# preshanth/rfi_toolbox

Hardware: AMD Instinct MI355X
Metric: training patches/sec (128x128x3) (higher is better)
Workload: dtype f32; 1 GPU; UNet(3,1,32) train step (fwd+BCE/dice+bwd+clip+Adam), batch 64/GPU x 128x128x3 NHWC, BASELINE configs[1] shape on the reference's U-Net (the '3-layer CNN' of configs[1] is not in the reference; its builder-defined form runs with --workload cnn3); global_batch=64, parallelism=dp1, params=7765985

## Files before the change

rfi_toolbox_amd/build.py:

```python
from __future__ import annotations

import os
import subprocess
import sys
from concurrent.futures import ThreadPoolExecutor

PKG = os.path.dirname(os.path.abspath(__file__))
ROOT = os.path.dirname(PKG)
CSRC = os.path.join(PKG, "csrc")
OBJ = os.path.join(ROOT, "build", "obj")
LIB = os.path.join(PKG, "librfi_hip.so")
HIPCC = os.environ.get("HIPCC", "/opt/rocm/bin/hipcc")
ARCH = "gfx950"

SOURCES = ["api.cpp", "api_ops.cpp", "model.cpp", "model_cnn.cpp", "model_planes.cpp", "model_resnet.cpp", "model_mask.cpp", "model_backbone.cpp", "model_mlp.cpp", "model_params.cpp", "elem_kernels.hip", "conv_direct.hip", "conv_mfma.hip",
           "wgrad_mfma.hip", "preprocess.hip", "synth.hip", "order_stats.hip", "planes_elem.hip", "conv_planes.hip", "conv_ws.hip", "conv_stem.hip", "gemm_ws.hip", "wgrad_ws.hip", "wgrad_stem.hip", "wgrad_planes.hip", "wgrad_split.hip", "detect_kernels.hip", "detect_sample.hip", "detect_infer.hip", "rpn_kernels.hip", "resnet_kernels.hip", "flag_stats.hip", "rfi_sim.hip", "stitch.hip", "dataset_norm.hip", "augment.hip", "sumthreshold.hip"]
HEADERS = ["common.hpp", "kernels.hpp", "model.hpp", "planes.hpp", "ws_common.hpp", "detect_sort.hpp", "select_common.hpp", os.path.join(ROOT, "include", "rfi_hip.h")]

COMMON = ["-O3", "-std=c++17", "-fPIC", f"--offload-arch={ARCH}", "-Wall", "-Wno-unused-function",
          "-ffp-contract=off"]
if os.environ.get("RFI_DIAG_STAMPS"):
    COMMON.append("-DRFI_DIAG_STAMPS=1")


def _newer(target, deps):
    if not os.path.exists(target):
        return True
    t = os.path.getmtime(target)
    return any(os.path.getmtime(d) > t for d in deps)


NO_SLP = {"elem_kernels.hip", "planes_elem.hip", "resnet_kernels.hip", "rpn_kernels.hip", "detect_kernels.hip",
          "preprocess.hip", "order_stats.hip", "synth.hip", "conv_direct.hip", "flag_stats.hip", "dataset_norm.hip", "augment.hip", "sumthreshold.hip",
          "conv_planes.hip", "wgrad_planes.hip", "wgrad_split.hip", "wgrad_mfma.hip", "conv_mfma.hip",
          "conv_ws.hip", "gemm_ws.hip", "wgrad_ws.hip", "conv_stem.hip", "wgrad_stem.hip"}


def flags_for(src):
    return ["-fno-slp-vectorize"] if src in NO_SLP else []


HAZARD_WINDOW = 20


def count_pk_f64_pairs(lines, window=HAZARD_WINDOW):
    import re
    n = 0
    for i, l in enumerate(lines):
        m = re.match(r"v_pk_\w+_f32\s+v\[(\d+):(\d+)\]", l)
        if not m:
            continue
        dst = set(range(int(m.group(1)), int(m.group(2)) + 1))
        for j in range(i + 1, min(i + 1 + window, len(lines))):
            if not dst:
                break
            c = re.match(r"v_cvt_f64_f32\w*\s+v\[\d+:\d+\],\s+v(\d+)", lines[j])
            if c and int(c.group(1)) in dst:
                n += 1
                break
            mv = re.match(r"v_mov_b32\w*\s+v(\d+),\s+v(\d+)\s*$", lines[j])
            copied = mv is not None and int(mv.group(2)) in dst
            w = re.match(r"v_\w+\s+v\[?(\d+)(?::(\d+))?\]?", lines[j])
            if w:
                dst -= set(range(int(w.group(1)), int(w.group(2) or w.group(1)) + 1))
            if copied:
                dst.add(int(mv.group(1)))
    return n


def isa_lines(path):
    return [l.strip() for l in open(path) if l.startswith("\t") and not l.startswith("\t.") and not l.startswith("\t;")]


def _compile(src, force, extra):
    import glob
    path = os.path.join(CSRC, src)
    obj = os.path.join(OBJ, src.replace(".", "_") + ".o")
    deps = [path] + [h if os.path.isabs(h) else os.path.join(CSRC, h) for h in HEADERS]
    if not force and not _newer(obj, deps):
        return obj, None
    device = src.endswith(".hip")
    cmd = [HIPCC, *COMMON, *flags_for(src), *extra, *(["-save-temps=obj"] if device else []), "-x", "hip", "-c", path, "-o", obj]
    r = subprocess.run(cmd, capture_output=True, text=True)
    if r.returncode != 0:
        raise RuntimeError(f"hipcc failed on {src}:\n{' '.join(cmd)}\n{r.stdout}\n{r.stderr}")
    if device:
        stem = os.path.join(OBJ, os.path.splitext(src)[0])
        asm = stem + "-hip-amdgcn-amd-amdhsa-gfx950.s"
        pairs = count_pk_f64_pairs(isa_lines(asm)) if os.path.exists(asm) else -1
        for f in glob.glob(stem + "-hip-amdgcn-amd-amdhsa-gfx950.*") + glob.glob(stem + "-host-x86_64-unknown-linux-gnu.*") + \
                glob.glob(stem + ".hip-hip-amdgcn-amd-amdhsa.hipfb"):
            os.remove(f)
        if pairs != 0:
            os.remove(obj)
            raise RuntimeError(f"{src}: " + ("no device ISA was produced to scan" if pairs < 0 else
                               f"{pairs} packed-fp32 -> v_cvt_f64_f32 pair(s) in the gfx950 ISA (a hazard on MI355X: see NO_SLP above); "
                               "build the source with -fno-slp-vectorize or form the product in float32 first"))
    return obj, r.stderr


# ... 22 lines not shown
```

rfi_toolbox_amd/csrc/conv_ws.hip:

```cpp
#include <algorithm>
#include <type_traits>
#include <vector>

#include <hip/hip_ext.h>

#include "ws_common.hpp"

namespace rfi {
namespace {

using namespace ws;

struct WsDev {
    const float* x;
    int x_ps;
    unsigned x_bytes;
    const float* scale;
    const float* shift;
    float slope;
    int N, H, W, Cin, Cout;
    const bf16_t* wB;
    int nkc, ncb;
    const float* bias;
    float* y;
    int y_ps;
    double* stats;
    int wide_epi;
    unsigned long long* stamps;
};

template <int P> constexpr int ROWB = 32 * P + 16;

template <int TB, int TH, int TW, int NTL, bool ADB, int P>
struct WsCfg {
    static constexpr int HH = TH + 2, HW = TW + 2, HPI = HH * HW, HP = TB * HPI;
    static constexpr int A_BYTES = (HP * ROWB<P> + 1023) & ~1023;
    static constexpr int NPIECE = 9 * NTL * P;
    static constexpr int B_BYTES = NPIECE * 1024;
    static constexpr int B_ITEMS = (NPIECE + 3) / 4;
    static constexpr int HALO_ITEMS = (HP * 4 + 255) / 256;
    static constexpr int B_OFF = (ADB ? 2 : 1) * A_BYTES;
    static constexpr int STAT_OFF = B_OFF + 2 * B_BYTES;
    static constexpr int STAT_BYTES = 4 * NTL * 64 * 2 * 8;
    static constexpr int EPI_WAVE_BYTES = 16 * 36 * 4;
    static constexpr bool WIDE_OK = STAT_OFF + 4 * EPI_WAVE_BYTES <= 160 * 1024;
    static constexpr int LDS_BYTES = STAT_OFF + ((STAT_BYTES > 4 * EPI_WAVE_BYTES || !WIDE_OK) ? STAT_BYTES : 4 * EPI_WAVE_BYTES);
    static_assert(TB * TH * TW == 256, "a tile is 256 output pixels");
    static_assert(32 % TW == 0 || TW % 32 == 0, "a 32-pixel block covers whole rows or a part of one");
    static_assert(LDS_BYTES <= 160 * 1024, "LDS budget");
};


template <int TB, int TH, int TW, int NTL, int XF, bool ADB, int P>
__global__ __launch_bounds__(512) void conv_ws_kernel(WsDev d) {
    using C = WsCfg<TB, TH, TW, NTL, ADB, P>;
    constexpr int RB = ROWB<P>;
    extern __shared__ __attribute__((aligned(16))) unsigned char smem[];
#ifdef RFI_DIAG_STAMPS
    unsigned long long st_[4] = {0, 0, 0, 0};
#endif
    const int tid = threadIdx.x;
    const int lane = tid & 63, wave = __builtin_amdgcn_readfirstlane(tid >> 6);

    const int tiles_x = (d.W + TW - 1) / TW, tiles_y = (d.H + TH - 1) / TH, tiles_b = (d.N + TB - 1) / TB;
    const int ntiles = tiles_b * tiles_y * tiles_x;
    const int GX = gridDim.x;
    int t_begin, t_count, j, gx;
    if (GX >= 8 && (GX & 7) == 0) {
        const int xcd = blockIdx.x & 7, q8 = ntiles >> 3, r8 = ntiles & 7;
        j = blockIdx.x >> 3;
        gx = GX >> 3;
        t_begin = xcd < r8 ? xcd * (q8 + 1) : r8 * (q8 + 1) + (xcd - r8) * q8;
        t_count = q8 + (xcd < r8 ? 1 : 0);
    } else {
        j = blockIdx.x; gx = GX; t_begin = 0; t_count = ntiles;
    }
    const int my_tiles = (j < t_count) ? (t_count - j + gx - 1) / gx : 0;
    const int cb0 = blockIdx.y * NTL, n0 = cb0 * 32;
    double* const st_out = d.stats ? d.stats + ((size_t)blockIdx.x * d.Cout + n0) * 2 : nullptr;
    if (my_tiles == 0) {
        if (st_out && tid < 32 * NTL && n0 + tid < d.Cout) st_out[tid * 2] = st_out[tid * 2 + 1] = 0.0;
        return;
    }
    struct Tile { int n, oy0, ox0; };
    auto tile_of = [&](int k) {
        const int t = t_begin + j + k * gx;
        Tile r;
        r.ox0 = (t % tiles_x) * TW;
        r.oy0 = ((t / tiles_x) % tiles_y) * TH;
        r.n = (t / (tiles_x * tiles_y)) * TB;
        return r;
    };
    const int nkc = d.nkc;
    const int nitems = my_tiles * nkc;
    double* const s_stat = reinterpret_cast<double*>(smem + C::STAT_OFF);

    if (wave >= 4) {
        const int ptid = tid - 256, pw = wave - 4;
        const unsigned q4b = (unsigned)(ptid & 3) * 16u;
        const __amdgpu_buffer_rsrc_t xrs = __builtin_amdgcn_make_buffer_rsrc(const_cast<float*>(d.x), 0, (int)d.x_bytes, 0x00020000);
        unsigned h_rc[C::HALO_ITEMS];
#pragma unroll
        for (int it = 0; it < C::HALO_ITEMS; ++it) {
            const int idx = ptid + it * 256, pix = idx >> 2;
            const int b = pix / C::HPI, rem = pix % C::HPI;
            h_rc[it] = idx < C::HP * 4 ? ((unsigned)b << 24) | ((unsigned)(rem / C::HW) << 12) | (unsigned)(rem % C::HW) : (0xfffu << 12);
        }
        unsigned voff[C::HALO_ITEMS];
        unsigned vmsk[C::HALO_ITEMS];
        auto setup_halo = [&](const Tile& t) {
#pragma unroll
            for (int it = 0; it < C::HALO_ITEMS; ++it) {
                const int n = t.n + (int)(h_rc[it] >> 24);
                const int iy = t.oy0 - 1 + (int)((h_rc[it] >> 12) & 0xfff), ix = t.ox0 - 1 + (int)(h_rc[it] & 0xfff);
                const bool ok = n < d.N && (unsigned)iy < (unsigned)d.H && (unsigned)ix < (unsigned)d.W;
                voff[it] = ok ? (unsigned)(((n * d.H + iy) * d.W + ix) * d.x_ps) * 4u + q4b : 0x80000000u;
                vmsk[it] = ok ? 0xffffffffu : 0u;
            }
        };
        u32x4 raw[C::HALO_ITEMS];
        f32x4 screg = {1.f, 1.f, 1.f, 1.f}, shreg = {0.f, 0.f, 0.f, 0.f};
        unsigned pl[C::HALO_ITEMS][2 * P];
        auto issue_loads = [&](int c0) {
            if constexpr (XF != 0) {
                screg = *reinterpret_cast<const f32x4*>(d.scale + c0 + (ptid & 3) * 4);
                shreg = *reinterpret_cast<const f32x4*>(d.shift + c0 + (ptid & 3) * 4);
            }
            __builtin_amdgcn_sched_barrier(0);
#pragma unroll
            for (int it = 0; it < C::HALO_ITEMS; ++it) raw[it] = __builtin_amdgcn_raw_buffer_load_b128(xrs, voff[it], c0 * 4, 0);
        };
        auto split_all = [&]() {
#pragma unroll
            for (int it = 0; it < C::HALO_ITEMS; ++it) {
                f32x4 v = __builtin_bit_cast(f32x4, raw[it]);
                if constexpr (XF != 0) {
#pragma unroll
                    for (int e = 0; e < 4; ++e) {
                        float t = v[e] * screg[e] + shreg[e];
                        if constexpr (XF == 1) asm("v_max_f32 %0, 0, %1" : "=v"(t) : "v"(t));
                        else t = __builtin_fmaxf(t, t * d.slope);
                        v[e] = __builtin_bit_cast(float, __builtin_bit_cast(unsigned, t) & vmsk[it]);
                    }
                }
                if constexpr (P == 3) {
                    split_pair(v.x, v.y, pl[it][0], pl[it][2], pl[it][4]);
                    split_pair(v.z, v.w, pl[it][1], pl[it][3], pl[it][5]);
                } else {
                    pl[it][0] = cvt_pair(v.x, v.y);
                    pl[it][1] = cvt_pair(v.z, v.w);
                }
            }
        };
        auto write_all = [&](int buf) {
            unsigned char* const sA = smem + buf * C::A_BYTES + (ptid >> 2) * RB + (ptid & 3) * 8;
#pragma unroll
            for (int it = 0; it < C::HALO_ITEMS; ++it) {
                if (ptid + it * 256 < C::HP * 4) {
                    unsigned char* row = sA + it * 64 * RB;
#pragma unroll
                    for (int p = 0; p < P; ++p) *reinterpret_cast<u32x2*>(row + 32 * p) = u32x2{pl[it][2 * p], pl[it][2 * p + 1]};
                }
            }
        };
// ... 253 lines not shown
                                        s_ep[(qi & 1) * 288 + (k + 4 * lh) * 36 + li] = v[0];
                                        s_ep[(qi & 1) * 288 + (k + 1 + 4 * lh) * 36 + li] = v[1];
                                        s1v[nt] += v;
                                        s2v[nt] = __builtin_elementwise_fma(v, v, s2v[nt]);
                                    }
                                }
                                if (qi > 0) {
                                    const int pq = qi - 1, nt = pq >> 3, mt = (pq >> 2) & 1;
                                    const int p = cw * 64 + mt * 32 + (pq & 3) * 8 + pl;
                                    const int b = p / (TH * TW), rr = p % (TH * TW);
                                    *reinterpret_cast<f32x4*>(d.y + tile_off + (unsigned)(((b * d.H + rr / TW) * d.W + rr % TW) * d.y_ps) +
                                                              (unsigned)(n0 + nt * 32 + c4)) = rq;
                                }
                            }
                        } else {
#pragma unroll
                            for (int e = 0; e < E; e += 2) {
                                const int nt = e / 32, mt = (e >> 4) & 1, r = e & 15;
                                const f32x2 v = f32x2{acc[mt][nt][r], acc[mt][nt][r + 1]} + f32x2{bias[nt], bias[nt]};
#pragma unroll
                                for (int k = 0; k < 2; ++k) {
                                    const int p = cw * 64 + mt * 32 + ((r + k) & 3) + 8 * ((r + k) >> 2);
                                    const int b = p / (TH * TW), rr = p % (TH * TW);
                                    d.y[tile_off + (unsigned)(((b * d.H + rr / TW) * d.W + rr % TW) * d.y_ps) + lane_off[nt]] = v[k];
                                }
                                s1v[nt] += v;
                                s2v[nt] = __builtin_elementwise_fma(v, v, s2v[nt]);
                            }
                        }
#pragma unroll
                        for (int nt = 0; nt < NTL; ++nt) {
                            s1[nt] += s1v[nt].x + s1v[nt].y;
                            s2[nt] += s2v[nt].x + s2v[nt].y;
                        }
                    } else {
                        epi_generic(acc, ct);
                    }
                    epi_finish();
                }
                cch = 0;
                ++ck;
                if (ck < my_tiles) ct = tile_of(ck);
            }
            WS_T(t4);
            wg_barrier();
            WS_T(t5);
            WS_ACC(0, t0, t1);
            WS_ACC(2, t1, t4);
            WS_ACC(1, t4, t5);
        }
        if constexpr (DEFER) {
            if (pend) {
                epi_generic(outr, pt);
                epi_finish();
            }
        }
        if (st_out) {
#pragma unroll
            for (int nt = 0; nt < NTL; ++nt) {
                s_stat[((cw * NTL + nt) * 64 + lane) * 2] = d1[nt];
                s_stat[((cw * NTL + nt) * 64 + lane) * 2 + 1] = d2[nt];
            }
        }
    }
#ifdef RFI_DIAG_STAMPS
    if (d.stamps && lane == 0) {
        unsigned long long* o = d.stamps + ((size_t)(blockIdx.y * gridDim.x + blockIdx.x) * 8 + wave) * 8;
        for (int i = 0; i < 4; ++i) o[i] = st_[i];
        o[4] = (unsigned long long)nitems;
    }
#endif
    if (st_out) {
        __syncthreads();
        if (tid < 32 * NTL && n0 + tid < d.Cout) {
            const int nt = tid >> 5, cl = tid & 31;
            double t1 = 0.0, t2 = 0.0;
#pragma unroll
            for (int w = 0; w < 4; ++w)
#pragma unroll
                for (int h = 0; h < 2; ++h) {
                    t1 += s_stat[((w * NTL + nt) * 64 + h * 32 + cl) * 2];
                    t2 += s_stat[((w * NTL + nt) * 64 + h * 32 + cl) * 2 + 1];
                }
            st_out[tid * 2] = t1;
            st_out[tid * 2 + 1] = t2;
        }
    }
}

template <int TB, int TH, int TW, int NTL, int XF, int P>
void launch_ws(rfi_ctx* ctx, ConvArgs& a, WsDev& d) {
    constexpr bool ADB = NTL == 1 || P == 1;
    using C = WsCfg<TB, TH, TW, NTL, ADB, P>;
    const int ntiles = (int)(cdiv(a.N, TB) * cdiv(a.H, TH) * cdiv(a.W, TW));
    const int ycols = (int)cdiv(d.ncb, NTL);
    const int gmax = std::max(8, 256 / ycols);
    const int tx = (int)cdiv(ntiles, 8);
    const int per = (int)cdiv(tx, std::max(1, gmax / 8));
    int GX = 8 * (int)cdiv(tx, per);
    if (ntiles < 8) GX = ntiles;
    if (a.stats && GX <= a.stats_max_records) a.stats_records = GX;
    else { a.stats = nullptr; a.stats_records = 0; }
    d.stats = a.stats;
    static PerDeviceOnce attr_once;
    attr_once.run(ctx->device, [&] {
        RFI_CHECK_HIP(hipFuncSetAttribute(reinterpret_cast<const void*>(&conv_ws_kernel<TB, TH, TW, NTL, XF, ADB, P>),
                                          hipFuncAttributeMaxDynamicSharedMemorySize, (int)C::LDS_BYTES));
    });
#ifdef RFI_DIAG_STAMPS
    {
        const size_t nw = (size_t)GX * ycols * 8;
        RFI_CHECK_HIP(hipMalloc(reinterpret_cast<void**>(&d.stamps), nw * 64));
        RFI_CHECK_HIP(hipMemsetAsync(d.stamps, 0, nw * 64, ctx->stream));
        hipLaunchKernelGGL((conv_ws_kernel<TB, TH, TW, NTL, XF, ADB, P>), dim3(GX, ycols), dim3(512), C::LDS_BYTES, ctx->stream, d);
        std::vector<unsigned long long> hs(nw * 8);
        RFI_CHECK_HIP(hipMemcpyAsync(hs.data(), d.stamps, nw * 64, hipMemcpyDeviceToHost, ctx->stream));
        RFI_CHECK_HIP(hipStreamSynchronize(ctx->stream));
        double c[5] = {0, 0, 0, 0, 0}, p[5] = {0, 0, 0, 0, 0};
        for (size_t w = 0; w < nw; ++w)
            for (int i = 0; i < 5; ++i) ((w & 7) < 4 ? c : p)[i] += (double)hs[w * 8 + i];
        std::fprintf(stderr, "[stamps] conv_ws<%d,%d,%d,%d,%d> N%d %dx%d %d->%d grid %dx%d items/wg %.1f | cycles per item: consumer mfma %.0f "
                     "epilogue %.0f barriers %.0f (+ in front of tap 8: %.0f) | producer work %.0f (split %.0f, dma wait %.0f) barriers+write %.0f\n", TB, TH, TW, NTL, XF,
                     a.N, a.H, a.W, a.Cin, a.Cout, GX, ycols, c[4] / (nw / 2), c[0] / c[4], c[2] / c[4], c[1] / c[4], c[3] / c[4], p[0] / p[4],
                     p[2] / p[4], p[3] / p[4], p[1] / p[4]);
        RFI_CHECK_HIP(hipFree(d.stamps));
        d.stamps = nullptr;
        return;
    }
#endif
    if (a.done) {
        hipExtLaunchKernelGGL((conv_ws_kernel<TB, TH, TW, NTL, XF, ADB, P>), dim3(GX, ycols), dim3(512), C::LDS_BYTES, ctx->stream, nullptr,
                              a.done, 0, d);
        a.done_used = true;
    } else {
        hipLaunchKernelGGL((conv_ws_kernel<TB, TH, TW, NTL, XF, ADB, P>), dim3(GX, ycols), dim3(512), C::LDS_BYTES, ctx->stream, d);
    }
    check_launch("conv_ws");
}

template <int NTL, int XF, int P>
void dispatch_ws(rfi_ctx* ctx, ConvArgs& a, WsDev& d) {
    if (a.W >= 32) launch_ws<1, 8, 32, NTL, XF, P>(ctx, a, d);
    else if (a.W >= 16) launch_ws<1, 16, 16, NTL, XF, P>(ctx, a, d);
    else launch_ws<4, 8, 8, NTL, XF, P>(ctx, a, d);
}
template <int NTL, int P>
void dispatch_xf(rfi_ctx* ctx, ConvArgs& a, WsDev& d, int xf) {
    if (xf == 0) dispatch_ws<NTL, 0, P>(ctx, a, d);
    else if (xf == 1) dispatch_ws<NTL, 1, P>(ctx, a, d);
    else dispatch_ws<NTL, 2, P>(ctx, a, d);
}

}

bool conv_ws_eligible(const ConvArgs& a) {
    if (!(a.R == 3 && a.S == 1 && a.pad == 1 && a.zgroups == 1 && a.fold == 0)) return false;
    if (a.Hin != a.H || a.Win != a.W || a.Hout != a.H || a.Wout != a.W) return false;
    if (a.osy != 1 || a.osx != 1 || a.ooy != 0 || a.oox != 0) return false;
    if (a.y16 || a.W < 8 || a.H < 8) return false;
    if (a.Cin % 16 != 0 || a.x.pstride % 4 != 0 || (reinterpret_cast<uintptr_t>(a.x.p) & 15)) return false;
    if (a.xf.scale && ((reinterpret_cast<uintptr_t>(a.xf.scale) & 15) || (reinterpret_cast<uintptr_t>(a.xf.shift) & 15))) return false;
    if ((int64_t)a.N * a.H * a.W * a.x.pstride * 4 >= (int64_t)1 << 31 || (int64_t)a.N * a.H * a.W * a.y.pstride >= (int64_t)1 << 31) return false;
    return true;
}

void launch_conv_ws(rfi_ctx* ctx, ConvArgs& a, const bf16_t* wB, int P) {
    RFI_REQUIRE(conv_ws_eligible(a), "conv_ws: shape not eligible");
    RFI_REQUIRE(P == 1 || P == 3, "conv_ws: planes must be 1 or 3");
    WsDev d;
    d.x = a.x.p; d.x_ps = a.x.pstride;
    d.x_bytes = (unsigned)((int64_t)a.N * a.H * a.W * a.x.pstride * 4);
    d.scale = a.xf.scale; d.shift = a.xf.shift;
    d.slope = a.xf.relu == 0 ? 1.0f : a.xf.slope;
    d.N = a.N; d.H = a.H; d.W = a.W; d.Cin = a.Cin; d.Cout = a.Cout;
    d.wB = wB;
    d.nkc = plane_chunks(a.Cin); d.ncb = (a.Cout + 31) / 32;
    RFI_REQUIRE((int64_t)wb_elems(9, a.Cout, a.Cin, 0, P) * 2 < ((int64_t)1 << 32), "conv_ws: filter tensor too large");
    d.bias = a.bias;
    d.y = a.y.p; d.y_ps = a.y.pstride;
    d.stats = nullptr;
    d.stamps = nullptr;
    d.wide_epi = a.y.pstride % 4 == 0 && (reinterpret_cast<uintptr_t>(a.y.p) & 15) == 0;
    const int64_t tiles = (a.W >= 16 ? (int64_t)a.N : cdiv(a.N, 4)) * cdiv(a.H, a.W >= 32 ? 8 : a.W >= 16 ? 16 : 8) * cdiv(a.W, a.W >= 32 ? 32 : a.W >= 16 ? 16 : 8);
    int ntl = 1;
    if (a.Cout > 32 && tiles * cdiv(d.ncb, 2) >= 224) ntl = 2;
    if (P == 1 && a.Cout > 64 && tiles * cdiv(d.ncb, 4) >= 224) ntl = 4;
// ... 21 lines not shown
```

rfi_toolbox_amd/csrc/elem_kernels.hip:

```cpp
#include <hip/hip_ext.h>

#include "kernels.hpp"

namespace rfi {

namespace {

constexpr int kBlock = 256;
constexpr int kFinCh = 2;
constexpr int kFinLanes = kBlock / kFinCh;

__device__ __forceinline__ double wave_sum(double v) {
#pragma unroll
    for (int o = 32; o > 0; o >>= 1) v += __shfl_down(v, o, 64);
    return v;
}

__device__ __forceinline__ double finish_sum(double v, double* red) {
#pragma unroll
    for (int o = 32; o >= kFinCh; o >>= 1) v += __shfl_xor(v, o, 64);
    const int wave = threadIdx.x >> 6, lane = threadIdx.x & 63;
    __syncthreads();
    if (lane < kFinCh) red[wave * kFinCh + lane] = v;
    __syncthreads();
    double t = 0;
    if (threadIdx.x < kFinCh)
        for (int w = 0; w < kBlock / 64; ++w) t += red[w * kFinCh + threadIdx.x];
    return t;
}

struct ChanGeom {
    int V;
    int CL, RL, cblocks;
    int64_t rows_per_block;
    int rblocks;
};

static ChanGeom chan_geom(int64_t M, int C, int max_rblocks, bool allow_vec = true, int force_v = 0) {
    ChanGeom g;
    g.V = force_v ? force_v : (allow_vec && C % 4 == 0) ? 4 : 1;
    const int lanes_needed = C / g.V;
    int cl = (g.V >= 4) ? 1 : 4;
    while (cl < lanes_needed && cl < 64) cl <<= 1;
    g.CL = cl;
    g.RL = kBlock / cl;
    g.cblocks = (int)cdiv(lanes_needed, cl);
    int64_t rpb = cdiv(M, max_rblocks);
    int64_t min_rows = (int64_t)g.RL * 8;
    if (rpb < min_rows) rpb = min_rows;
    rpb = cdiv(rpb, g.RL) * g.RL;
    g.rows_per_block = rpb;
    g.rblocks = (int)cdiv(M, rpb);
    return g;
}

template <int V>
__device__ __forceinline__ void ldv(const float* p, float (&v)[V]) {
    if constexpr (V == 4) {
        const float4 t = *reinterpret_cast<const float4*>(p);
        v[0] = t.x; v[1] = t.y; v[2] = t.z; v[3] = t.w;
    } else {
        v[0] = p[0];
    }
}
template <int V>
__device__ __forceinline__ void stv(float* p, const float (&v)[V]) {
    if constexpr (V == 4) *reinterpret_cast<float4*>(p) = make_float4(v[0], v[1], v[2], v[3]);
    else p[0] = v[0];
}
template <int V>
__device__ __forceinline__ void ldy(const void* y, int y16, int64_t idx, float (&v)[V]) {
    if (y16) {
        const unsigned short* q = static_cast<const unsigned short*>(y) + idx;
        if constexpr (V == 4) {
            const uint2 t = *reinterpret_cast<const uint2*>(q);
            v[0] = __builtin_bit_cast(float, t.x << 16); v[1] = __builtin_bit_cast(float, t.x & 0xffff0000u);
            v[2] = __builtin_bit_cast(float, t.y << 16); v[3] = __builtin_bit_cast(float, t.y & 0xffff0000u);
        } else {
            v[0] = __builtin_bit_cast(float, (unsigned)q[0] << 16);
        }
    } else {
        ldv<V>(static_cast<const float*>(y) + idx, v);
    }
}
__device__ __forceinline__ float ldy1(const void* y, int y16, int64_t idx) {
    float v[1];
    ldy<1>(y, y16, idx, v);
    return v[0];
}
__device__ __forceinline__ void round_store_bf16x4(unsigned short* p, float (&v)[4]) {
    unsigned short q[4];
#pragma unroll
    for (int e = 0; e < 4; ++e) {
        const __bf16 h = (__bf16)v[e];
        q[e] = __builtin_bit_cast(unsigned short, h);
        v[e] = (float)h;
    }
    *reinterpret_cast<uint2*>(p) = make_uint2((unsigned)q[0] | ((unsigned)q[1] << 16), (unsigned)q[2] | ((unsigned)q[3] << 16));
}
template <int V, int NQ>
__device__ __forceinline__ void row_lane_reduce(double (&acc)[NQ][V], double* red, int CL, int RL, int cl,
                                                int rl) {
#pragma unroll
// ... 18 lines not shown
                acc[q][v] = t0 + t1;
            }
    }
    if (NF > 1) {
        __syncthreads();
        if (rl > 0 && rl < NF) {
#pragma unroll
            for (int q = 0; q < NQ; ++q)
#pragma unroll
                for (int v = 0; v < V; ++v) red[(q * V + v) * kBlock + threadIdx.x] = acc[q][v];
        }
        __syncthreads();
        if (rl == 0) {
#pragma unroll
            for (int q = 0; q < NQ; ++q)
#pragma unroll
                for (int v = 0; v < V; ++v) {
                    double t = acc[q][v];
                    for (int j = 1; j < NF; ++j) t += red[(q * V + v) * kBlock + j * CL + cl];
                    acc[q][v] = t;
                }
        }
    }
}

__device__ __forceinline__ float act_f(float a, float slope) { return a > 0.0f ? a : (slope != 0.0f ? a * slope : 0.0f); }
__device__ __forceinline__ float dact_f(float z, float g, float slope) { return z > 0.0f ? g : g * slope; }

template <int V>
__global__ void bn_stats_kernel(const float* __restrict__ y, int64_t M, int C, int CL,
                                int64_t rows_per_block, double* __restrict__ partial) {
    __shared__ double red[2 * V * kBlock];
    const int RL = kBlock / CL;
    const int cl = threadIdx.x % CL, rl = threadIdx.x / CL;
    const int c = (blockIdx.y * CL + cl) * V;
    const int64_t r0 = (int64_t)blockIdx.x * rows_per_block;
    int64_t r1 = r0 + rows_per_block;
    if (r1 > M) r1 = M;
    double acc[2][V];
#pragma unroll
    for (int v = 0; v < V; ++v) acc[0][v] = acc[1][v] = 0;
    if (c < C) {
        for (int64_t r = r0 + rl; r < r1; r += RL) {
            float x[V];
            ldv<V>(y + r * C + c, x);
#pragma unroll
            for (int v = 0; v < V; ++v) {
                const double d = (double)x[v];
                acc[0][v] += d;
                acc[1][v] += d * d;
            }
        }
    }
    row_lane_reduce<V, 2>(acc, red, CL, RL, cl, rl);
    if (rl == 0 && c < C) {
#pragma unroll
        for (int v = 0; v < V; ++v) {
            partial[((int64_t)blockIdx.x * C + c + v) * 2 + 0] = acc[0][v];
            partial[((int64_t)blockIdx.x * C + c + v) * 2 + 1] = acc[1][v];
        }
    }
}

__global__ void bn_finalize_kernel(const double* __restrict__ partial, int records, int C,
                                   double count, const float* __restrict__ gamma,
                                   const float* __restrict__ beta, float* __restrict__ running_mean,
                                   float* __restrict__ running_var, int ema_repeats,
                                   float* __restrict__ mean_out, float* __restrict__ invstd_out,
                                   float* __restrict__ scale, float* __restrict__ shift,
                                   float* __restrict__ var_out) {
    __shared__ double red[2 * kBlock];
    const int cl = threadIdx.x & (kFinCh - 1), rl = threadIdx.x / kFinCh;
    const int c = blockIdx.x * kFinCh + cl;
    double s1 = 0, s2 = 0;
    if (c < C) {
        for (int r = rl; r < records; r += kFinLanes) {
            s1 += partial[((int64_t)r * C + c) * 2 + 0];
            s2 += partial[((int64_t)r * C + c) * 2 + 1];
        }
    }
    s1 = finish_sum(s1, red);
    s2 = finish_sum(s2, red);
    if (rl == 0 && c < C) {
        const double mean = s1 / count;
        double var = s2 / count - mean * mean;
        if (var < 0) var = 0;
        const double invstd = 1.0 / sqrt(var + 1e-5);
        const float meanf = (float)mean, invf = (float)invstd;
        mean_out[c] = meanf;
        invstd_out[c] = invf;
        if (var_out) var_out[c] = (float)var;
        const float sc = gamma[c] * invf;
        scale[c] = sc;
        shift[c] = beta[c] - meanf * sc;
        if (running_mean) {
            const double var_u = count > 1 ? var * (count / (count - 1.0)) : var;
            float rm = running_mean[c], rv = running_var[c];
            const float vuf = (float)var_u;
            for (int k = 0; k < ema_repeats; ++k) {
                rm = (1.0f - 0.1f) * rm + 0.1f * meanf;
                rv = (1.0f - 0.1f) * rv + 0.1f * vuf;
            }
            running_mean[c] = rm;
            running_var[c] = rv;
        }
    }
}

__global__ void bn_eval_coeffs_kernel(int C, const float* gamma, const float* beta, const float* rm,
                                      const float* rv, float* scale, float* shift) {
    int c = blockIdx.x * blockDim.x + threadIdx.x;
    if (c < C) {
        float inv = (float)(1.0 / sqrt((double)rv[c] + 1e-5));
        float sc = gamma[c] * inv;
        scale[c] = sc;
        shift[c] = beta[c] - rm[c] * sc;
    }
}

template <int V>
__global__ void bn_bwd_reduce_kernel(const void* __restrict__ da, int da16, const void* __restrict__ y, int y16, int64_t yps,
                                     int64_t M, int C, int CL, int64_t rows_per_block,
                                     const float* __restrict__ scale, const float* __restrict__ shift,
                                     const float* __restrict__ mean, const float* __restrict__ invstd,
                                     double* __restrict__ partial, float slope) {
    __shared__ double red[2 * V * kBlock];
    const int RL = kBlock / CL;
    const int cl = threadIdx.x % CL, rl = threadIdx.x / CL;
    const int c = (blockIdx.y * CL + cl) * V;
    const int64_t r0 = (int64_t)blockIdx.x * rows_per_block;
    int64_t r1 = r0 + rows_per_block;
    if (r1 > M) r1 = M;
    double acc[2][V];
#pragma unroll
    for (int v = 0; v < V; ++v) acc[0][v] = acc[1][v] = 0;
    if (c < C) {
        float sc[V], sh[V], mu[V], is[V];
        ldv<V>(scale + c, sc); ldv<V>(shift + c, sh); ldv<V>(mean + c, mu); ldv<V>(invstd + c, is);
        constexpr int U = 4;
        for (int64_t rb = r0 + rl; rb < r1; rb += (int64_t)U * RL) {
            float yv[U][V], dv[U][V];
#pragma unroll
            for (int k = 0; k < U; ++k) {
                const int64_t r = rb + (int64_t)k * RL;
                if (r < r1) {
                    ldy<V>(y, y16, r * yps + c, yv[k]);
                    ldy<V>(da, da16, r * C + c, dv[k]);
                }
            }
#pragma unroll
            for (int k = 0; k < U; ++k) {
                if (rb + (int64_t)k * RL < r1) {
#pragma unroll
                    for (int v = 0; v < V; ++v) {
                        const float dz = dact_f(yv[k][v] * sc[v] + sh[v], dv[k][v], slope);
                        const float xh = (yv[k][v] - mu[v]) * is[v];
                        acc[0][v] += (double)dz;
                        acc[1][v] += (double)dz * (double)xh;
                    }
                }
            }
        }
    }
    row_lane_reduce<V, 2>(acc, red, CL, RL, cl, rl);
    if (rl == 0 && c < C) {
#pragma unroll
        for (int v = 0; v < V; ++v) {
            partial[((int64_t)blockIdx.x * C + c + v) * 2 + 0] = acc[0][v];
            partial[((int64_t)blockIdx.x * C + c + v) * 2 + 1] = acc[1][v];
        }
    }
}

__device__ __forceinline__ void ld8h(const unsigned short* p, float (&v)[8]) {
    const uint4 t = *reinterpret_cast<const uint4*>(p);
    v[0] = __builtin_bit_cast(float, t.x << 16); v[1] = __builtin_bit_cast(float, t.x & 0xffff0000u);
    v[2] = __builtin_bit_cast(float, t.y << 16); v[3] = __builtin_bit_cast(float, t.y & 0xffff0000u);
    v[4] = __builtin_bit_cast(float, t.z << 16); v[5] = __builtin_bit_cast(float, t.z & 0xffff0000u);
    v[6] = __builtin_bit_cast(float, t.w << 16); v[7] = __builtin_bit_cast(float, t.w & 0xffff0000u);
}
__device__ __forceinline__ void ld8f(const float* p, float (&v)[8]) {
    const float4 a = *reinterpret_cast<const float4*>(p), b = *reinterpret_cast<const float4*>(p + 4);
    v[0] = a.x; v[1] = a.y; v[2] = a.z; v[3] = a.w; v[4] = b.x; v[5] = b.y; v[6] = b.z; v[7] = b.w;
}
__device__ __forceinline__ unsigned pack_bf16x2(float a, float b) {
    const __bf16 ha = (__bf16)a, hb = (__bf16)b;
    return (unsigned)__builtin_bit_cast(unsigned short, ha) | ((unsigned)__builtin_bit_cast(unsigned short, hb) << 16);
}
// ... 433 lines not shown
            if ((int)threadIdx.x < C4) {
#pragma unroll
                for (int v = 0; v < 4; ++v) {
                    double t1 = 0.0, t2 = 0.0;
                    for (int k = threadIdx.x; k < kBlock; k += C4) {
                        t1 += red[(2 * v) * kBlock + k];
                        t2 += red[(2 * v + 1) * kBlock + k];
                    }
                    records[((int64_t)blockIdx.x * C + c + v) * 2 + 0] = t1;
                    records[((int64_t)blockIdx.x * C + c + v) * 2 + 1] = t2;
                }
            }
        } else {
            const int per = C4 / kBlock;
#pragma unroll
            for (int v = 0; v < 4; ++v) {
                records[((int64_t)(blockIdx.x / per) * C + c + v) * 2 + 0] = s1[v];
                records[((int64_t)(blockIdx.x / per) * C + c + v) * 2 + 1] = s2[v];
            }
        }
    }
}

__global__ void copy_edge_kernel(int N, int H, int W, int C, const float* __restrict__ dskip,
                                 int dskip_ps, float* __restrict__ da) {
    const int64_t total = (int64_t)N * H * W * C;
    const int He = H & ~1, We = W & ~1;
    for (int64_t i = (int64_t)blockIdx.x * blockDim.x + threadIdx.x; i < total;
         i += (int64_t)gridDim.x * blockDim.x) {
        const int c = (int)(i % C);
        const int64_t pix = i / C;
        const int x = (int)(pix % W);
        const int yy = (int)((pix / W) % H);
        if (yy >= He || x >= We) da[pix * C + c] = dskip[pix * dskip_ps + c];
    }
}

__global__ void head_fwd_kernel(const float* __restrict__ y, int64_t M, int C,
                                const float* __restrict__ scale, const float* __restrict__ shift,
                                const float* __restrict__ w, const float* __restrict__ b, int Cout,
                                float* __restrict__ logits, float slope) {
    const int lane16 = threadIdx.x & 15;
    const int64_t m = ((int64_t)blockIdx.x * blockDim.x + threadIdx.x) >> 4;
    if (m >= M) return;
    for (int o = 0; o < Cout; ++o) {
        float acc = 0.0f;
        for (int c = lane16; c < C; c += 16) {
            float a = y[m * C + c] * scale[c] + shift[c];
            a = act_f(a, slope);
            acc += a * w[o * C + c];
        }
#pragma unroll
        for (int off = 8; off > 0; off >>= 1) acc += __shfl_down(acc, off, 16);
        if (lane16 == 0) logits[m * Cout + o] = acc + b[o];
    }
}

template <int L>
__global__ __launch_bounds__(256) void head_fwd_vec_kernel(const void* __restrict__ y, int y16, int64_t yps, int64_t M, int C,
                                                           const float* __restrict__ scale, const float* __restrict__ shift,
                                                           const float* __restrict__ w, const float* __restrict__ b, int Cout,
                                                           float* __restrict__ logits, float slope) {
    const int lane = threadIdx.x & (L - 1);
    const int64_t m = ((int64_t)blockIdx.x * blockDim.x + threadIdx.x) / L;
    if (m >= M) return;
    const int C4 = C >> 2;
    for (int o = 0; o < Cout; ++o) {
        float acc = 0.0f;
        for (int c4 = lane; c4 < C4; c4 += L) {
            float yv[4], sc[4], sh[4], wv[4];
            ldy<4>(y, y16, m * yps + 4 * c4, yv); ldv<4>(scale + 4 * c4, sc); ldv<4>(shift + 4 * c4, sh);
            ldv<4>(w + (int64_t)o * C + 4 * c4, wv);
#pragma unroll
            for (int v = 0; v < 4; ++v) acc += act_f(yv[v] * sc[v] + sh[v], slope) * wv[v];
        }
#pragma unroll
        for (int off = L / 2; off > 0; off >>= 1) acc += __shfl_down(acc, off, L);
        if (lane == 0) logits[m * Cout + o] = acc + b[o];
    }
}

__device__ __forceinline__ float sigmoidf_(float x) { return 1.0f / (1.0f + expf(-x)); }

__global__ void loss_reduce_kernel(const float* __restrict__ logits, const uint8_t* __restrict__ labels,
                                   int64_t count, double* __restrict__ partial) {
    __shared__ double red[4][kBlock / 64];
    double s[4] = {0, 0, 0, 0};
    for (int64_t i = (int64_t)blockIdx.x * blockDim.x + threadIdx.x; i < count;
         i += (int64_t)gridDim.x * blockDim.x) {
        const float x = logits[i];
        const float t = labels[i] ? 1.0f : 0.0f;
        const float bce = fmaxf(x, 0.0f) - x * t + log1pf(expf(-fabsf(x)));
        const float p = sigmoidf_(x);
        s[0] += (double)bce;
        s[1] += (double)(p * t);
        s[2] += (double)p;
        s[3] += (double)t;
    }
    const int wave = threadIdx.x >> 6, lane = threadIdx.x & 63;
#pragma unroll
    for (int k = 0; k < 4; ++k) {
        double v = wave_sum(s[k]);
        if (lane == 0) red[k][wave] = v;
    }
    __syncthreads();
    if (threadIdx.x < 4) {
        double v = 0;
        for (int wv = 0; wv < kBlock / 64; ++wv) v += red[threadIdx.x][wv];
        partial[(int64_t)blockIdx.x * 4 + threadIdx.x] = v;
    }
}

__global__ void loss_finish_kernel(const double* __restrict__ partial, int blocks, double count,
                                   double* __restrict__ sums4, float* __restrict__ loss_out) {
    __shared__ double red[4][kBlock / 64];
    double s[4] = {0, 0, 0, 0};
    for (int b = threadIdx.x; b < blocks; b += blockDim.x)
        for (int k = 0; k < 4; ++k) s[k] += partial[(int64_t)b * 4 + k];
    const int wave = threadIdx.x >> 6, lane = threadIdx.x & 63;
#pragma unroll
    for (int k = 0; k < 4; ++k) {
        double v = wave_sum(s[k]);
        if (lane == 0) red[k][wave] = v;
    }
    __syncthreads();
    if (threadIdx.x == 0) {
        double t[4];
        for (int k = 0; k < 4; ++k) {
            t[k] = 0;
            for (int wv = 0; wv < kBlock / 64; ++wv) t[k] += red[k][wv];
            sums4[k] = t[k];
        }
        const float bce = (float)(t[0] / count);
        const float inter = (float)t[1], sp = (float)t[2], st = (float)t[3];
        const float dice = 1.0f - (2.0f * inter + 1.0f) / (sp + st + 1.0f);
        loss_out[0] = bce + dice;
    }
}

__global__ void loss_bwd_kernel(const float* __restrict__ logits, const uint8_t* __restrict__ labels,
                                int64_t count, const double* __restrict__ sums4,
                                float* __restrict__ dlogits) {
    const float inter = (float)sums4[1], sp = (float)sums4[2], st = (float)sums4[3];
    const float D = sp + st + 1.0f;
    const float num = 2.0f * inter + 1.0f;
    const float invD2 = 1.0f / (D * D);
    const float invN = (float)(1.0 / (double)count);
    for (int64_t i = (int64_t)blockIdx.x * blockDim.x + threadIdx.x; i < count;
         i += (int64_t)gridDim.x * blockDim.x) {
        const float x = logits[i];
        const float t = labels[i] ? 1.0f : 0.0f;
        const float p = sigmoidf_(x);
        const float ddice = -(2.0f * t * D - num) * invD2;
        dlogits[i] = (p - t) * invN + ddice * p * (1.0f - p);
    }
}

__device__ __forceinline__ float focal_elem(float x, float t, float alpha, float gamma) {
    const float p = sigmoidf_(x);
    const float ce = fmaxf(x, 0.0f) - x * t + log1pf(expf(-fabsf(x)));
    const float pt = p * t + (1.0f - p) * (1.0f - t);
    const float at = alpha >= 0.0f ? alpha * t + (1.0f - alpha) * (1.0f - t) : 1.0f;
    return at * powf(1.0f - pt, gamma) * ce;
}
__global__ void focal_reduce_kernel(const float* __restrict__ logits, const uint8_t* __restrict__ labels,
                                    int64_t count, float alpha, float gamma, double* __restrict__ partial) {
    __shared__ double red[kBlock / 64];
    double s = 0;
    for (int64_t i = (int64_t)blockIdx.x * blockDim.x + threadIdx.x; i < count; i += (int64_t)gridDim.x * blockDim.x)
        s += (double)focal_elem(logits[i], labels[i] ? 1.0f : 0.0f, alpha, gamma);
    s = wave_sum(s);
    if ((threadIdx.x & 63) == 0) red[threadIdx.x >> 6] = s;
    __syncthreads();
    if (threadIdx.x == 0) {
        double t = 0;
        for (int k = 0; k < kBlock / 64; ++k) t += red[k];
        partial[blockIdx.x] = t;
    }
}
__global__ void focal_finish_kernel(const double* __restrict__ partial, int blocks, double count,
                                    float* __restrict__ loss_out) {
    __shared__ double red[kBlock / 64];
    double s = 0;
    for (int b = threadIdx.x; b < blocks; b += blockDim.x) s += partial[b];
    s = wave_sum(s);
    if ((threadIdx.x & 63) == 0) red[threadIdx.x >> 6] = s;
    __syncthreads();
    if (threadIdx.x == 0) {
        double t = 0;
        for (int k = 0; k < kBlock / 64; ++k) t += red[k];
        loss_out[0] = (float)(t / count);
    }
}
__global__ void focal_bwd_kernel(const float* __restrict__ logits, const uint8_t* __restrict__ labels, int64_t count,
                                 float alpha, float gamma, float* __restrict__ dlogits) {
    const float invN = (float)(1.0 / (double)count);
    for (int64_t i = (int64_t)blockIdx.x * blockDim.x + threadIdx.x; i < count; i += (int64_t)gridDim.x * blockDim.x) {
        const float x = logits[i];
        const bool pos = labels[i] != 0;
        const float p = sigmoidf_(x);
        const float sp_neg = fmaxf(-x, 0.0f) + log1pf(expf(-fabsf(x)));
        const float sp_pos = fmaxf(x, 0.0f) + log1pf(expf(-fabsf(x)));
        float g;
        if (pos) {
            const float a = alpha >= 0.0f ? alpha : 1.0f;
            g = a * powf(1.0f - p, gamma) * (gamma * p * (-sp_neg) - (1.0f - p));
        } else {
            const float a = alpha >= 0.0f ? 1.0f - alpha : 1.0f;
            g = a * powf(p, gamma) * (p - gamma * (1.0f - p) * (-sp_pos));
        }
        dlogits[i] = g * invN;
    }
}

__global__ void sigmoid_fwd_kernel(const float* __restrict__ z, int64_t n, float* __restrict__ x) {
    for (int64_t i = (int64_t)blockIdx.x * blockDim.x + threadIdx.x; i < n; i += (int64_t)gridDim.x * blockDim.x)
        x[i] = sigmoidf_(z[i]);
}
__global__ void sigmoid_bwd_kernel(const float* __restrict__ x, int64_t n, float* __restrict__ d) {
    for (int64_t i = (int64_t)blockIdx.x * blockDim.x + threadIdx.x; i < n; i += (int64_t)gridDim.x * blockDim.x) {
// ... 169 lines not shown
    }
}
__global__ void nhwc_to_nchw_kernel(const float* __restrict__ src, int N, int C, int H, int W,
                                    float* __restrict__ dst) {
    const int64_t total = (int64_t)N * C * H * W;
    for (int64_t i = (int64_t)blockIdx.x * blockDim.x + threadIdx.x; i < total;
         i += (int64_t)gridDim.x * blockDim.x) {
        const int x = (int)(i % W);
        int64_t t = i / W;
        const int yy = (int)(t % H);
        t /= H;
        const int c = (int)(t % C);
        const int n = (int)(t / C);
        dst[i] = src[(((int64_t)n * H + yy) * W + x) * C + c];
    }
}
__global__ void weight_to_dgrad_kernel(const float* __restrict__ wf, int taps, int Cout, int Cin,
                                       int flip, float* __restrict__ wd) {
    const int64_t total = (int64_t)taps * Cout * Cin;
    for (int64_t i = (int64_t)blockIdx.x * blockDim.x + threadIdx.x; i < total;
         i += (int64_t)gridDim.x * blockDim.x) {
        const int co = (int)(i % Cout);
        int64_t t = i / Cout;
        const int ci = (int)(t % Cin);
        const int tp = (int)(t / Cin);
        const int ts = flip ? (taps - 1 - tp) : tp;
        wd[i] = wf[((int64_t)ts * Cout + co) * Cin + ci];
    }
}
__global__ __launch_bounds__(256) void weight_to_dgrad_batched_kernel(const RelayoutDesc* __restrict__ descs, int n,
                                                                     const float* __restrict__ src, float* __restrict__ dst) {
    __shared__ float tile[32][33];
    const int64_t b = blockIdx.x;
    int l = 0;
    while (l + 1 < n && descs[l + 1].tile0 <= b) ++l;
    const RelayoutDesc d = descs[l];
    const float* __restrict__ wf = src + d.src_off;
    float* __restrict__ wd = dst + d.dst_off;
    const int tci = (d.cin + 31) / 32, tco = (d.cout + 31) / 32;
    const int t = (int)(b - d.tile0);
    const int tp = t / (tci * tco), r = t % (tci * tco);
    const int bco = r / tci, bci = r % tci;
    const int ts = d.flip ? (d.taps - 1 - tp) : tp;
    const int tx = threadIdx.x & 31, ty = threadIdx.x >> 5;
#pragma unroll
    for (int k = 0; k < 4; ++k) {
        const int co = bco * 32 + ty + 8 * k, ci = bci * 32 + tx;
        if (co < d.cout && ci < d.cin) tile[ty + 8 * k][tx] = wf[((int64_t)ts * d.cout + co) * d.cin + ci];
    }
    __syncthreads();
#pragma unroll
    for (int k = 0; k < 4; ++k) {
        const int ci = bci * 32 + ty + 8 * k, co = bco * 32 + tx;
        if (co < d.cout && ci < d.cin) wd[((int64_t)tp * d.cin + ci) * d.cout + co] = tile[tx][ty + 8 * k];
    }
}
__global__ void relu_bwd_kernel(float4* __restrict__ dA, const float4* __restrict__ Y, int64_t n4) {
    for (int64_t i = (int64_t)blockIdx.x * blockDim.x + threadIdx.x; i < n4;
         i += (int64_t)gridDim.x * blockDim.x) {
        float4 g = dA[i];
        const float4 y = Y[i];
        g.x = y.x > 0.0f ? g.x : 0.0f;
        g.y = y.y > 0.0f ? g.y : 0.0f;
        g.z = y.z > 0.0f ? g.z : 0.0f;
        g.w = y.w > 0.0f ? g.w : 0.0f;
        dA[i] = g;
    }
}
__global__ void pad_channels_kernel(const float* __restrict__ s, int64_t M, int c, int cp,
                                    float* __restrict__ d) {
    const int64_t total = M * cp;
    for (int64_t i = (int64_t)blockIdx.x * blockDim.x + threadIdx.x; i < total;
         i += (int64_t)gridDim.x * blockDim.x) {
        const int k = (int)(i % cp);
        d[i] = k < c ? s[(i / cp) * c + k] : 0.0f;
    }
}
__global__ void u8_to_f32_kernel(const uint8_t* __restrict__ s, int64_t n, float* __restrict__ d) {
    for (int64_t i = (int64_t)blockIdx.x * blockDim.x + threadIdx.x; i < n;
         i += (int64_t)gridDim.x * blockDim.x)
        d[i] = (float)s[i];
}

__global__ void sumsq_kernel(const float* __restrict__ g, int64_t n, double* __restrict__ partial) {
    __shared__ double red[kBlock / 64];
    double s = 0;
    const int64_t n4 = n >> 2;
    const float4* g4 = reinterpret_cast<const float4*>(g);
    for (int64_t i = (int64_t)blockIdx.x * blockDim.x + threadIdx.x; i < n4;
         i += (int64_t)gridDim.x * blockDim.x) {
        const float4 v = g4[i];
        s += (double)v.x * v.x + (double)v.y * v.y + (double)v.z * v.z + (double)v.w * v.w;
    }
    if (blockIdx.x == 0 && threadIdx.x < (n & 3)) {
        const float v = g[(n4 << 2) + threadIdx.x];
        s += (double)v * v;
    }
    s = wave_sum(s);
    if ((threadIdx.x & 63) == 0) red[threadIdx.x >> 6] = s;
    __syncthreads();
    if (threadIdx.x == 0) {
        double t = 0;
        for (int k = 0; k < kBlock / 64; ++k) t += red[k];
        partial[blockIdx.x] = t;
    }
}
__global__ void sumsq_finish_kernel(const double* __restrict__ partial, int blocks,
                                    double* __restrict__ out) {
    __shared__ double red[kBlock / 64];
    double s = 0;
    for (int b = threadIdx.x; b < blocks; b += blockDim.x) s += partial[b];
    s = wave_sum(s);
    if ((threadIdx.x & 63) == 0) red[threadIdx.x >> 6] = s;
    __syncthreads();
    if (threadIdx.x == 0) {
        double t = 0;
        for (int k = 0; k < kBlock / 64; ++k) t += red[k];
        out[0] = t;
    }
}

__global__ void adam_kernel(AdamArgs a) {
    const float norm = (float)sqrt(a.sumsq[0]) * a.grad_scale;
    float coef = a.max_norm / (norm + 1e-6f);
    coef = coef > 1.0f ? 1.0f : coef;
    if (a.max_norm <= 0.0f) coef = 1.0f;
    const float gs = a.grad_scale;
    for (int64_t i = (int64_t)blockIdx.x * blockDim.x + threadIdx.x; i < a.n;
         i += (int64_t)gridDim.x * blockDim.x) {
        const float p = a.p[i];
        float g = (a.g[i] * gs) * coef;
        g = __fmaf_rn(a.wd, p, g);
        const float m0 = a.m[i];
        const float m = __fmaf_rn(a.one_minus_beta1, g - m0, m0);
        const float v = __fmaf_rn(a.one_minus_beta2 * g, g, a.beta2 * a.v[i]);
        a.m[i] = m;
        a.v[i] = v;
        const float denom = sqrtf(v) / a.bc2_sqrt + a.eps;
        a.p[i] = p + (a.neg_step * m) / denom;
    }
    if (blockIdx.x == 0 && threadIdx.x == 0 && a.norm_out) a.norm_out[0] = norm;
}

__global__ void scale_inplace_kernel(float* __restrict__ x, int64_t n, float f) {
    for (int64_t i = (int64_t)blockIdx.x * blockDim.x + threadIdx.x; i < n; i += (int64_t)gridDim.x * blockDim.x) x[i] *= f;
}
__global__ void reduce_slabs_kernel(const float* __restrict__ slabs, int nslabs, int group, int kstride,
                                    int64_t n, float* __restrict__ out, int64_t out_rowstride) {
    const int base = blockIdx.y * group;
    int cnt = nslabs - base;
    if (cnt > group) cnt = group;
    for (int64_t i = (int64_t)blockIdx.x * blockDim.x + threadIdx.x; i < n;
         i += (int64_t)gridDim.x * blockDim.x) {
        float s = 0.0f;
        for (int k = 0; k < cnt; ++k) s += slabs[((int64_t)base + (int64_t)k) * kstride * n + i];
        out[(int64_t)blockIdx.y * out_rowstride * n + i] = s;
    }
}

__global__ __launch_bounds__(256) void reduce_slabs_vec4_kernel(const float* __restrict__ slabs, int nslabs, int group, int kstride,
                                                               int64_t n4, float* __restrict__ out, int64_t out_rowstride) {
    typedef float f32x4 __attribute__((ext_vector_type(4)));
    const int base = blockIdx.y * group;
    int cnt = nslabs - base;
    if (cnt > group) cnt = group;
    const f32x4* __restrict__ src = reinterpret_cast<const f32x4*>(slabs) + (int64_t)base * kstride * n4;
    f32x4* __restrict__ dst = reinterpret_cast<f32x4*>(out) + (int64_t)blockIdx.y * out_rowstride * n4;
    const int64_t step = (int64_t)kstride * n4;
    for (int64_t i = (int64_t)blockIdx.x * blockDim.x + threadIdx.x; i < n4; i += (int64_t)gridDim.x * blockDim.x) {
        f32x4 s = {0.f, 0.f, 0.f, 0.f};
        int k = 0;
        for (; k + 8 <= cnt; k += 8) {
            f32x4 v[8];
#pragma unroll
            for (int u = 0; u < 8; ++u) v[u] = __builtin_nontemporal_load(src + (int64_t)(k + u) * step + i);
#pragma unroll
            for (int u = 0; u < 8; ++u) s += v[u];
        }
        for (; k < cnt; ++k) s += __builtin_nontemporal_load(src + (int64_t)k * step + i);
        dst[i] = s;
    }
}

static int grid_for(int64_t total, int cap = 256 * 16) {
    int64_t b = cdiv(total, kBlock);
    if (b > cap) b = cap;
    if (b < 1) b = 1;
    return (int)b;
}

constexpr int kMaxRowBlocks = 1024;

}
// ... 223 lines not shown
           !((reinterpret_cast<uintptr_t>(y.p) | reinterpret_cast<uintptr_t>(scale) | reinterpret_cast<uintptr_t>(shift) |
              reinterpret_cast<uintptr_t>(dskip.p) | reinterpret_cast<uintptr_t>(dpool) | reinterpret_cast<uintptr_t>(da)) & 15);
}
int launch_pool_bwd_merge_sums(rfi_ctx* ctx, YRef y, int N, int H, int W, int C, const float* scale,
                               const float* shift, const float* mean, const float* invstd, YRef dskip, YRef dpool,
                               float* da, float slope, float* partial_ws, unsigned short* da16) {
    if (!pool_vec_ok(y, C, scale, shift, dskip, dpool, da16 ? reinterpret_cast<const float*>(da16) : da) || dpool.stride(C) != C ||
        (reinterpret_cast<uintptr_t>(da16) & 7) ||
        ((reinterpret_cast<uintptr_t>(mean) | reinterpret_cast<uintptr_t>(invstd)) & 15))
        return 0;
    const int C4 = C / 4;
    const int64_t total = (int64_t)N * (H / 2) * (W / 2) * C4;
    const bool small = C4 <= kBlock && kBlock % C4 == 0, wide = C4 > kBlock && C4 % kBlock == 0;
    if ((H & 1) || (W & 1) || !(small || wide) || total < (int64_t)kBlock * 16) return 0;
    int grid = grid_for(total, kMaxRowBlocks);
    int records = grid;
    if (wide) {
        const int per = C4 / kBlock;
        grid = std::max(per, grid / per * per);
        records = grid / per;
    }
    if ((int64_t)grid * kBlock > total) return 0;
    ProfScope ps(ctx, FAM_ELEMWISE, 0, (double)N * H * W * C * (y.bf16 ? 10 : 12) + (double)total * (dpool.bf16 ? 8 : 16));
    hipLaunchKernelGGL(pool_bwd_merge_vec_kernel<true>, dim3(grid), dim3(kBlock), 0, ctx->stream, y.p, y.bf16, y.stride(C), N, H, W,
                       C, scale, shift, mean, invstd, dskip.p, dskip.bf16, (int)dskip.stride(C), dpool.p, dpool.bf16, da, slope, reinterpret_cast<double*>(partial_ws), da16);
    check_launch("pool_bwd_merge_sums");
    return records;
}

void launch_pool_bwd_merge(rfi_ctx* ctx, YRef y, int N, int H, int W, int C,
                           const float* scale, const float* shift, YRef dskip, YRef dpool,
                           float* da, float slope, unsigned short* da16) {
    const bool vec = pool_vec_ok(y, C, scale, shift, dskip, dpool, da16 ? reinterpret_cast<const float*>(da16) : da) && dpool.stride(C) == C &&
                     !(reinterpret_cast<uintptr_t>(da16) & 7);
    RFI_REQUIRE(vec || !(dpool.bf16 || da16 || dskip.bf16), "pool_bwd_merge: bfloat16 gradient tensors need C % 4 == 0 and aligned tensors");
    RFI_REQUIRE(!dskip.bf16 || !((H & 1) || (W & 1)), "pool_bwd_merge: a bfloat16 skip gradient needs even H and W");
    RFI_REQUIRE(!da16 || !((H & 1) || (W & 1)), "pool_bwd_merge: a bfloat16 output needs even H and W");
    const int64_t total = (int64_t)N * (H / 2) * (W / 2) * C;
    {
        ProfScope ps(ctx, FAM_ELEMWISE, 0, (double)N * H * W * C * (y.bf16 ? 10 : 12) + (double)total * (dpool.bf16 ? 2 : 4));
        if (vec)
            hipLaunchKernelGGL(pool_bwd_merge_vec_kernel<false>, dim3(grid_for(total / 4)), dim3(kBlock), 0, ctx->stream, y.p, y.bf16,
                               y.stride(C), N, H, W, C, scale, shift, nullptr, nullptr, dskip.p, dskip.bf16, (int)dskip.stride(C), dpool.p, dpool.bf16, da, slope, nullptr, da16);
        else
            hipLaunchKernelGGL(pool_bwd_merge_kernel, dim3(grid_for(total)), dim3(kBlock), 0, ctx->stream, y.p, y.bf16, y.stride(C),
                               N, H, W, C, scale, shift, static_cast<const float*>(dskip.p), (int)dskip.stride(C), static_cast<const float*>(dpool.p), da, slope);
        check_launch("pool_bwd_merge");
    }
    if ((H & 1) || (W & 1)) {
        ProfScope ps(ctx, FAM_ELEMWISE);
        hipLaunchKernelGGL(copy_edge_kernel, dim3(grid_for((int64_t)N * H * W * C)), dim3(kBlock), 0,
                           ctx->stream, N, H, W, C, static_cast<const float*>(dskip.p), (int)dskip.stride(C), da);
        check_launch("copy_edge");
    }
}

void launch_head_fwd(rfi_ctx* ctx, YRef yr, int64_t M, int C, const float* scale,
                     const float* shift, const float* w, const float* b, int Cout, float* logits, float slope) {
    ProfScope ps(ctx, FAM_ELEMWISE, 2.0 * M * C * Cout, (double)M * C * (yr.bf16 ? 2 : 4) + (double)M * Cout * 4);
    const bool vec = C % 4 == 0 && !((reinterpret_cast<uintptr_t>(yr.p) | reinterpret_cast<uintptr_t>(scale) |
                                      reinterpret_cast<uintptr_t>(shift) | reinterpret_cast<uintptr_t>(w)) & 15) && yr.stride(C) % 4 == 0;
    RFI_REQUIRE(vec || !yr.bf16, "head_fwd: a bfloat16 input needs C % 4 == 0");
    const float* y = static_cast<const float*>(yr.p);
    if (vec) {
        int L = 1;
        while (L * 2 <= C / 4 && L < 16) L *= 2;
        const unsigned blocks = (unsigned)cdiv(M * L, kBlock);
#define RFI_HF(L_) hipLaunchKernelGGL(head_fwd_vec_kernel<L_>, dim3(blocks), dim3(kBlock), 0, ctx->stream, yr.p, yr.bf16, yr.stride(C), M, C, scale, shift, w, b, Cout, logits, slope)
        if (L == 16) RFI_HF(16); else if (L == 8) RFI_HF(8); else if (L == 4) RFI_HF(4); else if (L == 2) RFI_HF(2); else RFI_HF(1);
#undef RFI_HF
    } else {
        const int64_t threads = M * 16;
        hipLaunchKernelGGL(head_fwd_kernel, dim3((unsigned)cdiv(threads, kBlock)), dim3(kBlock), 0,
                           ctx->stream, y, M, C, scale, shift, w, b, Cout, logits, slope);
    }
    check_launch("head_fwd");
}

size_t loss_ws_doubles(int64_t count) {
    (void)count;
    return 4 * 1024 + 8;
}
void launch_loss_reduce(rfi_ctx* ctx, const float* logits, const uint8_t* labels, int64_t count,
                        double* partial_ws, double* sums4, float* loss_out) {
    int blocks = grid_for(count, 1024);
    {
        ProfScope ps(ctx, FAM_ELEMWISE, 0, (double)count * 5);
        hipLaunchKernelGGL(loss_reduce_kernel, dim3(blocks), dim3(kBlock), 0, ctx->stream, logits, labels,
                           count, partial_ws);
        check_launch("loss_reduce");
    }
    {
        ProfScope ps(ctx, FAM_ELEMWISE);
        hipLaunchKernelGGL(loss_finish_kernel, dim3(1), dim3(kBlock), 0, ctx->stream, partial_ws, blocks,
                           (double)count, sums4, loss_out);
        check_launch("loss_finish");
    }
}
void launch_focal_reduce(rfi_ctx* ctx, const float* logits, const uint8_t* labels, int64_t count, float alpha,
                         float gamma, double* partial_ws, float* loss_out) {
    int blocks = grid_for(count, 1024);
    {
        ProfScope ps(ctx, FAM_ELEMWISE, 0, (double)count * 5);
        hipLaunchKernelGGL(focal_reduce_kernel, dim3(blocks), dim3(kBlock), 0, ctx->stream, logits, labels, count,
                           alpha, gamma, partial_ws);
        check_launch("focal_reduce");
    }
    {
        ProfScope ps(ctx, FAM_ELEMWISE);
        hipLaunchKernelGGL(focal_finish_kernel, dim3(1), dim3(kBlock), 0, ctx->stream, partial_ws, blocks,
                           (double)count, loss_out);
        check_launch("focal_finish");
    }
}
void launch_focal_bwd(rfi_ctx* ctx, const float* logits, const uint8_t* labels, int64_t count, float alpha,
                      float gamma, float* dlogits) {
    ProfScope ps(ctx, FAM_ELEMWISE, 0, (double)count * 9);
    hipLaunchKernelGGL(focal_bwd_kernel, dim3(grid_for(count)), dim3(kBlock), 0, ctx->stream, logits, labels,
                       count, alpha, gamma, dlogits);
    check_launch("focal_bwd");
}
void launch_loss_bwd(rfi_ctx* ctx, const float* logits, const uint8_t* labels, int64_t count,
                     const double* sums4, float* dlogits) {
    ProfScope ps(ctx, FAM_ELEMWISE, 0, (double)count * 9);
    hipLaunchKernelGGL(loss_bwd_kernel, dim3(grid_for(count)), dim3(kBlock), 0, ctx->stream, logits,
                       labels, count, sums4, dlogits);
    check_launch("loss_bwd");
}

void launch_sigmoid_fwd(rfi_ctx* ctx, const float* z, int64_t n, float* x) {
    ProfScope ps(ctx, FAM_ELEMWISE, 0, (double)n * 8);
    hipLaunchKernelGGL(sigmoid_fwd_kernel, dim3(grid_for(n)), dim3(kBlock), 0, ctx->stream, z, n, x);
    check_launch("sigmoid_fwd");
}
void launch_sigmoid_bwd(rfi_ctx* ctx, const float* x, int64_t n, float* d_inout) {
    ProfScope ps(ctx, FAM_ELEMWISE, 0, (double)n * 12);
    hipLaunchKernelGGL(sigmoid_bwd_kernel, dim3(grid_for(n)), dim3(kBlock), 0, ctx->stream, x, n, d_inout);
    check_launch("sigmoid_bwd");
}

size_t head_bwd_ws_floats(int64_t M, int C, int Cout) {
    (void)M;
    return (size_t)kMaxRowBlocks * ((size_t)Cout * C + Cout) * 2;
}
int launch_head_bwd(rfi_ctx* ctx, YRef yr, int64_t M, int C, const float* scale,
                    const float* shift, const float* w, int Cout, const float* dlogits, float* da,
                    float* partial_ws, float* dw, float* db, float slope, const float* bn_mean, const float* bn_invstd,
                    float* bn_records_ws, unsigned short* da16, bool* skip_da, bool finish) {
    const bool may_skip = skip_da && *skip_da;
    if (skip_da) *skip_da = false;
    int bn_records = 0;
    const bool vec = C % 4 == 0 && !((reinterpret_cast<uintptr_t>(yr.p) | reinterpret_cast<uintptr_t>(da) |
                                      reinterpret_cast<uintptr_t>(scale) | reinterpret_cast<uintptr_t>(shift) |
                                      reinterpret_cast<uintptr_t>(w)) & 15) && yr.stride(C) % 4 == 0;
    RFI_REQUIRE(vec || !yr.bf16, "head_bwd: a bfloat16 input needs C % 4 == 0");
    RFI_REQUIRE(finish || vec, "head_bwd: deferred finishing needs the vector path (C % 4 == 0, 16-byte aligned tensors)");
    RFI_REQUIRE(!da16 || (vec && Cout == 1 && !(reinterpret_cast<uintptr_t>(da16) & 7)), "head_bwd: a bfloat16 gradient tensor needs C % 4 == 0 and one output channel");
    const float* y = static_cast<const float*>(yr.p);
    ChanGeom g = geom_rows(M, C, vec);
    {
        ProfScope ps(ctx, FAM_ELEMWISE, 4.0 * M * C * Cout, (double)M * C * (yr.bf16 ? 6 : 8));
        if (vec) {
            const bool sums = bn_records_ws && bn_mean && bn_invstd && Cout == 1 &&
                              !((reinterpret_cast<uintptr_t>(bn_mean) | reinterpret_cast<uintptr_t>(bn_invstd)) & 15);
            hipLaunchKernelGGL(head_bwd_vec_kernel, dim3(g.rblocks, g.cblocks), dim3(kBlock), 0, ctx->stream, yr.p, yr.bf16,
                               yr.stride(C), M, C, g.CL, g.rows_per_block, scale, shift, w, Cout, dlogits, da,
                               reinterpret_cast<double*>(partial_ws), slope, bn_mean, bn_invstd,
                               sums ? reinterpret_cast<double*>(bn_records_ws) : nullptr, da16, (sums && may_skip && !da16) ? 0 : 1);
            if (sums) bn_records = g.rblocks;
            if (sums && may_skip && !da16) *skip_da = true;
        }
        else
            hipLaunchKernelGGL(head_bwd_kernel, dim3(g.rblocks, g.cblocks), dim3(kBlock), 0, ctx->stream, y,
                               M, C, g.CL, g.rows_per_block, scale, shift, w, Cout, dlogits, da,
                               reinterpret_cast<double*>(partial_ws), slope);
        check_launch("head_bwd");
    }
    if (finish) {
        const int n = Cout * C + Cout;
        ProfScope ps(ctx, FAM_REDUCE);
        hipLaunchKernelGGL(finish_channel_sum_kernel, dim3((int)cdiv(Cout * C, kFinCh)), dim3(kBlock), 0,
                           ctx->stream, reinterpret_cast<const double*>(partial_ws), g.rblocks, (int64_t)n, Cout * C, dw);
        check_launch("head_bwd_finish_dw");
    }
    if (finish) {
        const int n = Cout * C + Cout;
        ProfScope ps(ctx, FAM_REDUCE);
        hipLaunchKernelGGL(finish_channel_sum_kernel, dim3((int)cdiv(Cout, kFinCh)), dim3(kBlock), 0,
                           ctx->stream, reinterpret_cast<const double*>(partial_ws) + (size_t)Cout * C,
                           g.rblocks, (int64_t)n, Cout, db);
        check_launch("head_bwd_finish_db");
    }
    return bn_records;
}

void launch_nchw_to_nhwc(rfi_ctx* ctx, const float* src, int N, int C, int H, int W, float* dst) {
    const int64_t total = (int64_t)N * C * H * W;
    ProfScope ps(ctx, FAM_ELEMWISE, 0, (double)total * 8);
    hipLaunchKernelGGL(nchw_to_nhwc_kernel, dim3(grid_for(total)), dim3(kBlock), 0, ctx->stream, src, N,
                       C, H, W, dst);
    check_launch("nchw_to_nhwc");
}
void launch_nhwc_to_nchw(rfi_ctx* ctx, const float* src, int N, int C, int H, int W, float* dst) {
    const int64_t total = (int64_t)N * C * H * W;
    ProfScope ps(ctx, FAM_ELEMWISE, 0, (double)total * 8);
    hipLaunchKernelGGL(nhwc_to_nchw_kernel, dim3(grid_for(total)), dim3(kBlock), 0, ctx->stream, src, N,
                       C, H, W, dst);
    check_launch("nhwc_to_nchw");
}
void launch_weight_to_dgrad(rfi_ctx* ctx, const float* wf, int taps, int Cout, int Cin, int flip,
                            float* wd) {
    const int64_t total = (int64_t)taps * Cout * Cin;
    ProfScope ps(ctx, FAM_ELEMWISE, 0, (double)total * 8);
    hipLaunchKernelGGL(weight_to_dgrad_kernel, dim3(grid_for(total)), dim3(kBlock), 0, ctx->stream, wf,
                       taps, Cout, Cin, flip, wd);
    check_launch("weight_to_dgrad");
}
int64_t relayout_assign_tiles(RelayoutDesc* descs, int n) {
    int64_t t = 0;
    for (int i = 0; i < n; ++i) {
        descs[i].tile0 = t;
        t += (int64_t)descs[i].taps * ((descs[i].cout + 31) / 32) * ((descs[i].cin + 31) / 32);
    }
    return t;
}
void launch_weight_to_dgrad_batched(rfi_ctx* ctx, const RelayoutDesc* descs_dev, int n, const float* src,
                                    float* dst, double total_bytes, int64_t total_tiles) {
    RFI_REQUIRE(total_tiles > 0 && total_tiles < ((int64_t)1 << 31), "weight_to_dgrad_batched: bad tile count");
    ProfScope ps(ctx, FAM_ELEMWISE, 0, total_bytes);
    hipLaunchKernelGGL(weight_to_dgrad_batched_kernel, dim3((unsigned)total_tiles), dim3(256), 0, ctx->stream, descs_dev, n,
                       src, dst);
    check_launch("weight_to_dgrad_batched");
}
void launch_relu_bwd(rfi_ctx* ctx, float* dA, const float* Y, int64_t n) {
    RFI_REQUIRE(n % 4 == 0, "relu_bwd: element count must be a multiple of 4");
    ProfScope ps(ctx, FAM_ELEMWISE, 0, (double)n * 12);
    hipLaunchKernelGGL(relu_bwd_kernel, dim3(grid_for(n / 4)), dim3(kBlock), 0, ctx->stream,
                       reinterpret_cast<float4*>(dA), reinterpret_cast<const float4*>(Y), n / 4);
    check_launch("relu_bwd");
}
void launch_pad_channels(rfi_ctx* ctx, const float* src, int64_t M, int c, int cp, float* dst) {
    ProfScope ps(ctx, FAM_ELEMWISE, 0, (double)M * (c + cp) * 4);
    hipLaunchKernelGGL(pad_channels_kernel, dim3(grid_for(M * cp)), dim3(kBlock), 0, ctx->stream, src, M, c,
                       cp, dst);
    check_launch("pad_channels");
}
void launch_u8_to_f32(rfi_ctx* ctx, const uint8_t* src, int64_t n, float* dst) {
    ProfScope ps(ctx, FAM_ELEMWISE, 0, (double)n * 5);
    hipLaunchKernelGGL(u8_to_f32_kernel, dim3(grid_for(n)), dim3(kBlock), 0, ctx->stream, src, n, dst);
    check_launch("u8_to_f32");
}

size_t sumsq_ws_doubles(int64_t n) {
    (void)n;
    return 1024 + 8;
}
void launch_sumsq(rfi_ctx* ctx, const float* g, int64_t n, double* partial_ws, double* sumsq) {
    int blocks = grid_for(n / 4 + 1, 1024);
    {
        ProfScope ps(ctx, FAM_OPTIM, 0, (double)n * 4);
        hipLaunchKernelGGL(sumsq_kernel, dim3(blocks), dim3(kBlock), 0, ctx->stream, g, n, partial_ws);
        check_launch("sumsq");
    }
    {
        ProfScope ps(ctx, FAM_OPTIM);
        hipLaunchKernelGGL(sumsq_finish_kernel, dim3(1), dim3(kBlock), 0, ctx->stream, partial_ws, blocks,
                           sumsq);
        check_launch("sumsq_finish");
    }
}
void launch_adam(rfi_ctx* ctx, const AdamArgs& a) {
    ProfScope ps(ctx, FAM_OPTIM, 0, (double)a.n * 28);
    hipLaunchKernelGGL(adam_kernel, dim3(grid_for(a.n)), dim3(kBlock), 0, ctx->stream, a);
    check_launch("adam");
}

void launch_scale_inplace(rfi_ctx* ctx, float* x, int64_t n, float f) {
    if (n <= 0) return;
    ProfScope ps(ctx, FAM_COMM, 0, (double)n * 8);
    hipLaunchKernelGGL(scale_inplace_kernel, dim3(grid_for(n)), dim3(kBlock), 0, ctx->stream, x, n, f);
    check_launch("scale_inplace");
}
void launch_reduce_slabs(rfi_ctx* ctx, const float* slabs, int nslabs, int64_t n, float* out) {
    float* s = const_cast<float*>(slabs);
    int count = nslabs;
    int stride = 1;
    const bool vec = n % 4 == 0 && !((reinterpret_cast<uintptr_t>(slabs) | reinterpret_cast<uintptr_t>(out)) & 15);
    while (count > 32) {
        const int groups = (int)cdiv(count, 32);
        ProfScope ps(ctx, FAM_REDUCE, 0, (double)n * 4 * (count + groups));
        if (vec)
            hipLaunchKernelGGL(reduce_slabs_vec4_kernel, dim3(grid_for(n / 4, 1024), groups), dim3(kBlock), 0, ctx->stream, s, count, 32,
                               stride, n / 4, s, (int64_t)32 * stride);
        else
        hipLaunchKernelGGL(reduce_slabs_kernel, dim3(grid_for(n, 1024), groups), dim3(kBlock), 0,
                           ctx->stream, s, count, 32, stride, n, s, (int64_t)32 * stride);
        check_launch("reduce_slabs_fold");
        count = groups;
        stride *= 32;
    }
    ProfScope ps(ctx, FAM_REDUCE, 0, (double)n * 4 * (count + 1));
    if (vec)
        hipLaunchKernelGGL(reduce_slabs_vec4_kernel, dim3(grid_for(n / 4, 1024), 1), dim3(kBlock), 0, ctx->stream, s, count, 32, stride,
                           n / 4, out, (int64_t)0);
    else
    hipLaunchKernelGGL(reduce_slabs_kernel, dim3(grid_for(n, 1024), 1), dim3(kBlock), 0, ctx->stream, s,
                       count, 32, stride, n, out, (int64_t)0);
    check_launch("reduce_slabs");
}

}
```

rfi_toolbox_amd/csrc/kernels.hpp:

```cpp
#pragma once
#include "common.hpp"

namespace rfi {

struct InXform {
    const float* scale = nullptr;
    const float* shift = nullptr;
    int relu = 0;
    float slope = 0.0f;
};
static inline InXform act_xform(const float* scale, const float* shift, float slope) {
    return InXform{scale, shift, slope != 0.0f ? 2 : 1, slope};
}

struct View {
    const float* p = nullptr;
    int pstride = 0;
};
struct MutView {
    float* p = nullptr;
    int pstride = 0;
};

struct ConvArgs {
    View x;
    int N = 0, H = 0, W = 0;
    int Hin = 0, Win = 0;
    int Cin = 0, Cout = 0;
    const float* w = nullptr;
    const float* w3 = nullptr;
    const unsigned short* wB3 = nullptr;
    const unsigned short* wB1 = nullptr;
    const float* bias = nullptr;
    MutView y;
    int Hout = 0, Wout = 0;
    int osy = 1, osx = 1;
    int ooy = 0, oox = 0;
    int R = 3, S = 1, pad = 1;
    int zgroups = 1;
    unsigned short* y16 = nullptr;
    int fold = 0;
    InXform xf;
    double algo_flops = -1;
    bool bf16 = false;
    bool bf16x3 = false;
    int planes = 0;
    double* stats = nullptr;
    int stats_max_records = 0;
    int stats_records = 0;
    hipEvent_t done = nullptr;
    bool done_used = false;
#ifdef RFI_DIAG_STAMPS
    unsigned long long* stamps = nullptr;
#endif
};

enum ConvImpl { IMPL_AUTO = 0, IMPL_DIRECT = 1, IMPL_MFMA = 2, IMPL_MFMA_BF16 = 3, IMPL_MFMA_BF16X3 = 4,
                IMPL_PLANES_X3 = 5, IMPL_PLANES_BF16 = 6, IMPL_WS_X3 = 7, IMPL_WS_BF16 = 8 };
bool conv_ws_eligible(const ConvArgs& a);
void launch_conv_ws(rfi_ctx* ctx, ConvArgs& a, const unsigned short* wB, int P);
bool gemm_ws_eligible(const ConvArgs& a);
void launch_gemm_ws(rfi_ctx* ctx, ConvArgs& a, const unsigned short* wB3);

bool conv_mfma_eligible(const ConvArgs& a);
size_t weights_x3_floats(int taps, int Cout, int Cin);
void launch_weights_to_x3(rfi_ctx* ctx, const float* w, int taps, int Cout, int Cin, float* out);
struct X3Desc { const float* src; float* dst; int64_t rows; int Cin; int nchunks; };
void launch_weights_to_x3_batched(rfi_ctx* ctx, const X3Desc* descs_dev, int n, double total_bytes);
bool conv_stem_eligible(const ConvArgs& a);
void launch_conv_stem(rfi_ctx* ctx, ConvArgs& a);
void launch_conv(rfi_ctx* ctx, ConvArgs& a, int impl = IMPL_AUTO);

struct WgradArgs {
    View xop, yop;
    InXform xf_x, xf_y;
    int N = 0, H = 0, W = 0;
    int Hx = 0, Wx = 0;
    int Cx = 0, Cy = 0;
    int R = 3, S = 1, pad = 1;
    float* dw = nullptr;
    int64_t tap_stride = 0;
    int sy = 0, sx = 0;
    float* slab = nullptr;
    size_t slab_floats = 0;
    double algo_flops = -1;
    bool bf16 = false;
    bool bf16x3 = false;
    int planes = 0;
};
size_t wgrad_slab_floats(const WgradArgs& a, int impl);
bool wgrad_ws_eligible(const WgradArgs& a);
void launch_wgrad_ws(rfi_ctx* ctx, const WgradArgs& a);
size_t wgrad_ws_slab_floats(const WgradArgs& a);
bool wgrad_stem_eligible(const WgradArgs& a);
void launch_wgrad_stem(rfi_ctx* ctx, const WgradArgs& a);
void launch_wgrad(rfi_ctx* ctx, const WgradArgs& a, int impl = IMPL_AUTO);

struct YRef {
    const void* p = nullptr;
    int bf16 = 0;
    int64_t ps = 0;
    YRef(const float* f) : p(f) {}
    YRef(float* f) : p(f) {}
    YRef(const float* f, int64_t pstride) : p(f), ps(pstride) {}
    YRef(const unsigned short* h, int64_t pstride) : p(h), bf16(1), ps(pstride) {}
    YRef(View v) : p(v.p), ps(v.pstride) {}
    int64_t stride(int C) const { return ps ? ps : C; }
};

size_t bn_stats_ws_floats(int C);
void launch_bn_stats(rfi_ctx* ctx, const float* y, int64_t M, int C, float* partial_ws);
void launch_bn_finalize(rfi_ctx* ctx, const float* partial_ws, int64_t M, int C, const float* gamma,
                        const float* beta, float* running_mean, float* running_var,
                        int ema_repeats, float* mean, float* invstd, float* scale, float* shift,
                        float* var_out, int records = 0,
                        hipEvent_t done = nullptr);
void launch_bn_eval_coeffs(rfi_ctx* ctx, int C, const float* gamma, const float* beta,
                           const float* running_mean, const float* running_var, float* scale,
                           float* shift);
void launch_bn_bwd_reduce(rfi_ctx* ctx, YRef da, YRef y, int64_t M, int C,
                          const float* scale, const float* shift, const float* mean,
                          const float* invstd, float* partial_ws, float* c1, float* c2,
                          float* dgamma, float* dbeta, float slope = 0.0f);
size_t bn_bwd_ws_floats(int64_t M, int C);
void launch_bn_bwd_finalize_records(rfi_ctx* ctx, const float* partial_ws, int records, int64_t M, int C, float* c1,
                                    float* c2, float* dgamma, float* dbeta);
void launch_bn_bwd_apply(rfi_ctx* ctx, YRef da_inout, YRef y, int64_t M, int C,
                         const float* scale, const float* shift, const float* mean,
                         const float* invstd, const float* gamma, const float* c1, const float* c2,
                         float* partial_ws, float* dbias, float slope = 0.0f,
                         unsigned short* planes_out = nullptr, int64_t planes_pstride = 0, int planes_P = 0,
                         hipEvent_t done = nullptr, bool finish_dbias = true, const float* head_dl = nullptr,
                         const float* head_w = nullptr);
void launch_bn_bwd_apply_finish(rfi_ctx* ctx, const float* partial_ws, int64_t M, int C, float* dbias);
struct FinishSumDesc { const double* partial; int records; int64_t stride; int count; float* out; };
int bn_bwd_apply_records(int64_t M, int C);
void launch_finish_channel_sums_batched(rfi_ctx* ctx, const FinishSumDesc* descs_dev, int n, int max_count);

void launch_bn_relu_pool(rfi_ctx* ctx, const float* y, int N, int H, int W, int C,
                         const float* scale, const float* shift, MutView skip, float* pooled, float slope = 0.0f);
void launch_pool_bwd_merge(rfi_ctx* ctx, YRef y, int N, int H, int W, int C,
                           const float* scale, const float* shift, YRef dskip, YRef dpool,
                           float* da, float slope = 0.0f, unsigned short* da16 = nullptr);
int launch_pool_bwd_merge_sums(rfi_ctx* ctx, YRef y, int N, int H, int W, int C, const float* scale,
                               const float* shift, const float* mean, const float* invstd, YRef dskip, YRef dpool,
                               float* da, float slope, float* partial_ws, unsigned short* da16 = nullptr);
void launch_head_fwd(rfi_ctx* ctx, YRef y, int64_t M, int C, const float* scale,
                     const float* shift, const float* w, const float* b, int Cout, float* logits,
                     float slope = 0.0f);
void launch_sigmoid_fwd(rfi_ctx* ctx, const float* z, int64_t n, float* x);
void launch_sigmoid_bwd(rfi_ctx* ctx, const float* x, int64_t n, float* d_inout);
void launch_loss_reduce(rfi_ctx* ctx, const float* logits, const uint8_t* labels, int64_t count,
                        double* partial_ws, double* sums4, float* loss_out);
size_t loss_ws_doubles(int64_t count);
void launch_loss_bwd(rfi_ctx* ctx, const float* logits, const uint8_t* labels, int64_t count,
                     const double* sums4, float* dlogits);
void launch_focal_reduce(rfi_ctx* ctx, const float* logits, const uint8_t* labels, int64_t count, float alpha,
                         float gamma, double* partial_ws, float* loss_out);
void launch_focal_bwd(rfi_ctx* ctx, const float* logits, const uint8_t* labels, int64_t count, float alpha,
                      float gamma, float* dlogits);
int launch_head_bwd(rfi_ctx* ctx, YRef y, int64_t M, int C, const float* scale,
                    const float* shift, const float* w, int Cout, const float* dlogits, float* da,
                    float* partial_ws, float* dw, float* db, float slope = 0.0f, const float* bn_mean = nullptr,
                    const float* bn_invstd = nullptr, float* bn_records_ws = nullptr, unsigned short* da16 = nullptr,
                    bool* skip_da = nullptr, bool finish = true);
size_t head_bwd_ws_floats(int64_t M, int C, int Cout);
void launch_channel_sum(rfi_ctx* ctx, View v, int64_t M, int C, float* partial_ws, float* out, bool finish = true);
void launch_channel_sum(rfi_ctx* ctx, YRef v, int64_t M, int C, float* partial_ws, float* out, bool finish = true);
size_t channel_sum_ws_floats(int64_t M, int C);

void launch_nchw_to_nhwc(rfi_ctx* ctx, const float* src, int N, int C, int H, int W, float* dst);
void launch_nhwc_to_nchw(rfi_ctx* ctx, const float* src, int N, int C, int H, int W, float* dst);
void launch_weight_to_dgrad(rfi_ctx* ctx, const float* wf, int taps, int Cout, int Cin, int flip,
                            float* wd);
struct RelayoutDesc {
    int64_t src_off, dst_off;
    int taps, cout, cin, flip;
    int64_t tile0 = 0;
};
int64_t relayout_assign_tiles(RelayoutDesc* descs, int n);
void launch_weight_to_dgrad_batched(rfi_ctx* ctx, const RelayoutDesc* descs_dev, int n, const float* src,
                                    float* dst, double total_bytes, int64_t total_tiles);
void launch_u8_to_f32(rfi_ctx* ctx, const uint8_t* src, int64_t n, float* dst);
void launch_relu_bwd(rfi_ctx* ctx, float* dA, const float* Y, int64_t n);
void launch_pad_channels(rfi_ctx* ctx, const float* src, int64_t M, int c, int cp, float* dst);

void launch_sumsq(rfi_ctx* ctx, const float* g, int64_t n, double* partial_ws, double* sumsq);
size_t sumsq_ws_doubles(int64_t n);
struct AdamArgs {
    float* p; float* g; float* m; float* v; int64_t n;
    float beta2, eps, wd, max_norm, grad_scale;
    float one_minus_beta1, one_minus_beta2;
    float neg_step, bc2_sqrt;
    const double* sumsq;
    float* norm_out;
};
void launch_adam(rfi_ctx* ctx, const AdamArgs& a);

void launch_preprocess(rfi_ctx* ctx, const void* patches, int dtype, int n, int ph, int pw,
                       float* minmax_ws, float* out_nhwc, const rfi_patch_src* table_dev = nullptr, int C = 0,
                       int T = 0);
void launch_patch_median(rfi_ctx* ctx, const double* v, int n, int per, bool absdev, const double* centre,
                         bool finite_only, double* out, int* cnt_out, bool f32 = false);
void launch_scale_by_median(rfi_ctx* ctx, double* v, int n, int per, const double* med, bool f32 = false);
void launch_stretch(rfi_ctx* ctx, double* v, int64_t total, int kind, bool f32 = false);
void launch_replace_inf(rfi_ctx* ctx, double* v, int n, int per, const double* mad, const int* nfinite);
void launch_mad_flags(rfi_ctx* ctx, const double* v, int n, int per, const double* med, const double* mad,
                      double sigma, uint8_t* flags, bool f32 = false);
void launch_narrow_f32(rfi_ctx* ctx, const double* src, int64_t total, float* dst);
void launch_to_abs_f64(rfi_ctx* ctx, const void* src, int dtype, int64_t total, double* dst);
void launch_synth(rfi_ctx* ctx, unsigned long long seed, int n_samples, int n_pol, int C, int T, double noise,
                  int bandpass, int order, double corr, const rfi_event* events_dev, const int* offsets_dev,
                  int out_dtype, void* planes, uint8_t* flags);
void launch_gather_labels(rfi_ctx* ctx, const uint8_t* flags, const rfi_patch_src* table_dev, int C, int T, int n,
                          int ps, uint8_t* out);
void launch_patch_any_flag(rfi_ctx* ctx, const uint8_t* flags, const rfi_patch_src* table_dev, int C, int T, int n,
                           int ps, unsigned* any_out);
void launch_confusion(rfi_ctx* ctx, const void* pred, int pred_dtype, const void* truth,
                      int truth_dtype, int64_t count, unsigned long long* counts3);
void launch_threshold(rfi_ctx* ctx, const float* logits, int64_t count, float threshold,
                      uint8_t* mask);
int64_t tiling_patches_per_plane(int C, int T, const rfi_tiling& tiling);
void check_tiling(const rfi_tiling& tiling);
void launch_stitch(rfi_ctx* ctx, const float* values, int kind, int n_planes, int C, int T, const rfi_tiling& tiling,
                   int combine, float threshold, uint8_t* flags, float* prob);
size_t flag_stats_ws_bytes();
void launch_flag_stats(rfi_ctx* ctx, const void* src, int dtype, int64_t n, const uint8_t* flags, int views,
                       bool medians, void* ws, void* mag, rfi_flag_stats* out_dev);
struct norm_chunk { const void* ptr; int64_t start; };
size_t norm_stats_ws_bytes(int pops, int64_t seg);
int norm_stats_passes(bool f32, bool quantiles);
void launch_norm_stats(rfi_ctx* ctx, const norm_chunk* chunks_dev, int n_chunks, bool f32, int64_t seg, int pops,
                       bool quantiles, const int64_t* ranks6, void* ws, rfi_norm_stats* out_dev);
void launch_norm_apply(rfi_ctx* ctx, const void* src, int dtype, bool src_nhwc, int n, int64_t px, double centre, double scale,
                       const double* params_dev, float* dst, bool dst_nhwc);
void augment_params_host(const rfi_augment_config& cfg, uint64_t call, int n, int h, int w, int32_t* gates, double* inv);
void launch_augment(rfi_ctx* ctx, const float* x, const uint8_t* y, int n, int h, int w, int c, const rfi_augment_config& cfg,
                    uint64_t call, float* x_out, uint8_t* y_out);
void sumthreshold_ladder_host(const rfi_sumthreshold_config& cfg, double sigma, int iteration, double* chi);
size_t st_state_bytes(int planes);
int st_max_window();
void launch_st_pass(rfi_ctx* ctx, const float* X, const float* B, const uint8_t* Fin, uint8_t* Fout, int planes, int C, int T, int M,
                    int axis, const double* center, const double* chi, int pstride, const int* done, int dstride);
void launch_st_smooth(rfi_ctx* ctx, const float* X, const uint8_t* F, int planes, int C, int T, const double* wt, int ht,
                      const double* wf, int hf, double* nd, float* B);
void launch_st_sir(rfi_ctx* ctx, const uint8_t* Fin, uint8_t* Fout, int planes, int C, int T, int axis, int q, int* ws);
void launch_sumthreshold_flag(rfi_ctx* ctx, const void* src, int dtype, const uint8_t* prior, int planes, int C, int T,
                              const rfi_sumthreshold_config& cfg, const double* wt, const double* wf, float* X, float* B, uint8_t* Fa,
                              uint8_t* Fb, double* nd, void* state, uint8_t* out);
void launch_rfi_sim(rfi_ctx* ctx, unsigned long long seed, unsigned first_sample, int n_samples,
                    const rfi_sim_params& p, const double* power_dev, int layout, void* out, uint8_t* mask,
                    rfi_sim_event* events, double* baseline_out);

void launch_scale_inplace(rfi_ctx* ctx, float* x, int64_t n, float f);
void launch_roi_align_fwd(rfi_ctx* ctx, const float* x, int N, int H, int W, int C, const float* rois, int R, float scale,
                          int PH, int PW, int sampling_ratio, bool aligned, float* out);
void launch_roi_align_bwd(rfi_ctx* ctx, const float* dout, int N, int H, int W, int C, const float* rois, int R, float scale,
                          int PH, int PW, int sr, bool aligned, float* dx);
void launch_mask_targets(rfi_ctx* ctx, const unsigned char* masks, int G, int H, int W, const float* rois, int R, int PH, int PW,
                         int sr, unsigned char* out);
void launch_anchor_match_batched(rfi_ctx* ctx, const float* anchors, int64_t n, int64_t anchor_stride, const int* anchor_count,
                                 const float* gt, int B, int Gmax, const int* gt_count, float hi, float lo, bool low_quality,
                                 float* best_ws, signed char* labels, int* matched, float* targets);
void launch_nms_batched(rfi_ctx* ctx, const float* boxes, const int* count, int B, int K, float thr, unsigned char* keep);
void launch_fpn_merge_fwd(rfi_ctx* ctx, const float* lateral, const float* top, int N, int H, int W, int C, float* out);
void launch_fpn_merge_bwd_top(rfi_ctx* ctx, const float* dout, int N, int H, int W, int C, float* dtop);

void launch_box_decode(rfi_ctx* ctx, const float* anchors, int64_t n_anchors, const float* deltas, int64_t n, float clip_h,
                       float clip_w, float* out);
void launch_nms_mask(rfi_ctx* ctx, const float* boxes, int n, float thr, unsigned long long* mask);
// ... 61 lines not shown
```

rfi_toolbox_amd/csrc/model.cpp:

```cpp
#include "model.hpp"

#include <cmath>
#include <cstdlib>
#include <random>

using namespace rfi;

namespace rfi {

void DevBuf::ensure(rfi_ctx* c, size_t floats) {
    if (floats <= n && p) return;
    if (p) c->release(p);
    ctx = c;
    p = static_cast<float*>(c->alloc(floats * sizeof(float)));
    n = floats;
}
void DevBuf::free() {
    if (p && ctx) ctx->release(p);
    p = nullptr;
    n = 0;
}

}

rfi_model::~rfi_model() {
    if (!ctx) return;
    ctx->activate();
    for (auto& b : bufs) b.free();
    if (ws_pool) ctx->release(ws_pool);
    if (ws_descs) ctx->release(ws_descs);
    for (float* p : {params, grads, adam_m, adam_v, chan_pool, wd_pool, w3_pool, grad_acc})
        if (p) ctx->release(p);
    if (relayout_descs) ctx->release(relayout_descs);
    if (x3_descs) ctx->release(x3_descs);
    if (d_sums) ctx->release(d_sums);
    if (d_scalars) ctx->release(d_scalars);
    if (wd_ready) (void)hipEventDestroy(wd_ready);
    if (lazy_ev) (void)hipEventDestroy(lazy_ev);
}

UNetModel::~UNetModel() {
    if (!ctx) return;
    ctx->activate();
    for (auto& b : pl) b.free();
    for (void* p : {(void*)wb_pool, wb_descs, (void*)dbias_pool, dbias_descs, (void*)rs_wpool, (void*)rs_cls_pool})
        if (p) ctx->release(p);
}

void UNetModel::build() {
    if (resnet_encoder) return build_resnet();
    RFI_REQUIRE(in_ch > 0 && out_ch > 0 && feat > 0, "UNet: channel counts must be positive");
    RFI_REQUIRE(depth >= 1 && depth <= 6, "UNet: depth must be in [1,6]");
    const int D = depth;
    i_bott = 2 * D;
    auto add = [&](const std::string& prefix, int conv_idx, int bn_idx, int cin, int cout, int ema, int lvl) {
        ConvBN c;
        c.conv_name = prefix + "." + std::to_string(conv_idx);
        c.bn_name = prefix + "." + std::to_string(bn_idx);
        c.cin = cin;
        c.cin_p = convs.empty() ? (int)align4((size_t)cin) : cin;
        c.cout = cout;
        c.ema_repeats = ema;
        c.level = lvl;
        add_conv(c);
    };
    int cin = in_ch;
    for (int l = 1; l <= D; ++l) {
        const int cout = feat << (l - 1);
        const std::string p = "encoder" + std::to_string(l) + ".conv.conv";
        add(p, 0, 1, cin, cout, 2, l);
        add(p, 3, 4, cout, cout, 2, l);
        cin = cout;
    }
    add("bottleneck.conv", 0, 1, cin, cin * 2, 1, D + 1);
    add("bottleneck.conv", 3, 4, cin * 2, cin * 2, 1, D + 1);
    cin *= 2;
    for (int l = D; l >= 1; --l) {
        const int cout = feat << (l - 1);
        add_up("decoder" + std::to_string(l) + ".up", cin, cout);
        const std::string p = "decoder" + std::to_string(l) + ".conv.conv";
        add(p, 0, 1, cin, cout, 1, l);
        add(p, 3, 4, cout, cout, 1, l);
        cin = cout;
    }
    add_head("final_conv", feat);
    alloc_state();
}

void UNetModel::set_planes(int P) {
    if (P == planesP) return;
    ctx->activate();
    RFI_CHECK_HIP(hipStreamSynchronize(ctx->main_stream));
    RFI_CHECK_HIP(hipStreamSynchronize(ctx->side_stream));
    for (auto& b : pl) b.free();
    if (wb_pool) { ctx->release(wb_pool); wb_pool = nullptr; }
    if (wb_descs) { ctx->release(wb_descs); wb_descs = nullptr; }
    planesP = P;
    wd_dirty = true;
    pN = 0;
}

void rfi_model::prepare(int n, int h, int w) {
    RFI_REQUIRE(n > 0 && h > 0 && w > 0, "forward: empty batch or image");
    join_pending_side();
    if (ctx->stream != ctx->main_stream) {
        ctx->stream = ctx->main_stream;
        RFI_CHECK_HIP(hipStreamSynchronize(ctx->side_stream));
        side_seq = 0;
    }
    if (side_seq != 0 || ctx->fork_ring_used != 0 || ctx->bucket_ev_used != 0 || pend_hi > pend_lo) {
        RFI_CHECK_HIP(hipStreamSynchronize(ctx->main_stream));
        RFI_CHECK_HIP(hipStreamSynchronize(ctx->side_stream));
        if (ctx->comm_stream) RFI_CHECK_HIP(hipStreamSynchronize(ctx->comm_stream));
        side_seq = 0;
        ctx->fork_ring_used = 0;
        ctx->bucket_ev_used = 0;
        pend_lo = pend_hi = 0;
    }
    prepare_shape(n, h, w);
// ... 289 lines not shown
                c.ws3d = ws_pool + o;
                const size_t e = wb_elems(9, c.cin_p, c.cout, 0, P);
                o += e + 32;
                hdg.push_back(WBDesc{c.wd, c.ws3d, 9, c.cin_p, c.cout, {c.cout, 0}, P});
                ws_by_w[c.wd] = c.ws3d;
                ws_bytes += 2.0 * e + 4.0 * 9 * c.cin_p * c.cout;
            }
            if (one_ok(c)) {
                const size_t ef = wb_elems(1, c.cout, c.cin_p, 0, P), ed = wb_elems(1, c.cin_p, c.cout, 0, P);
                hd.push_back(WBDesc{params + c.w_off, ws_pool + o, 1, c.cout, c.cin_p, {c.cin_p, 0}, P});
                ws_by_w[params + c.w_off] = ws_pool + o;
                o += ef + 32;
                hdg.push_back(WBDesc{c.wd, ws_pool + o, 1, c.cin_p, c.cout, {c.cout, 0}, P});
                ws_by_w[c.wd] = ws_pool + o;
                o += ed + 32;
                ws_bytes_fwd += 2.0 * ef + 4.0 * c.cin_p * c.cout;
                ws_bytes += 2.0 * ed + 4.0 * c.cin_p * c.cout;
            }
        }
        for (UpConv& u : ups) {
            if (!up_ok(u)) continue;
            const size_t ef = wb_elems(1, 4 * u.cout, u.cin, 0, P), ed = wb_elems(4, u.cin, u.cout, 0, P);
            hd.push_back(WBDesc{params + u.w_off, ws_pool + o, 1, 4 * u.cout, u.cin, {u.cin, 0}, P});
            ws_by_w[params + u.w_off] = ws_pool + o;
            o += ef + 32;
            hdg.push_back(WBDesc{u.wd, ws_pool + o, 4, u.cin, u.cout, {u.cout, 0}, P});
            ws_by_w[u.wd] = ws_pool + o;
            o += ed + 32;
            ws_bytes_fwd += 2.0 * ef + 4.0 * 4 * u.cin * u.cout;
            ws_bytes += 2.0 * ed + 4.0 * 4 * u.cin * u.cout;
        }
        ws_n_fwd = (int)hd.size();
        ws_bytes += ws_bytes_fwd;
        hd.insert(hd.end(), hdg.begin(), hdg.end());
        ws_n = (int)hd.size();
        ws_descs = ctx->upload_table(hd.data(), hd.size() * sizeof(WBDesc));
    }
    const WBDesc* descs = static_cast<const WBDesc*>(ws_descs);
    if (which == 0 && ws_n) launch_weights_to_wb(ctx, descs, ws_n, ws_bytes);
    if (which == 1 && ws_n_fwd) launch_weights_to_wb(ctx, descs, ws_n_fwd, ws_bytes_fwd);
    if (which == 2 && ws_n > ws_n_fwd) launch_weights_to_wb(ctx, descs + ws_n_fwd, ws_n - ws_n_fwd, ws_bytes - ws_bytes_fwd);
}

ConvArgs rfi_model::conv_same(View x, InXform xf, Shape s, int R, int pad, int cin, int cout, const float* w, const float* w3,
                              const float* bias, float* y) const {
    ConvArgs a;
    a.x = x;
    a.N = s.N; a.H = s.H; a.W = s.W; a.Hin = s.H; a.Win = s.W;
    a.Cin = cin; a.Cout = cout;
    set_filters(a, w, w3);
    a.bias = bias;
    a.y = MutView{y, cout};
    a.Hout = s.H; a.Wout = s.W;
    a.R = R; a.S = 1; a.pad = pad;
    a.xf = xf;
    return a;
}

WgradArgs rfi_model::wgrad_same(View x, InXform xf_x, const float* dy, Shape s, int R, int pad, int cin, int cout,
                                float* dw) const {
    WgradArgs wa;
    wa.xop = x;
    wa.yop = View{dy, cout};
    wa.xf_x = xf_x;
    wa.N = s.N; wa.H = s.H; wa.W = s.W; wa.Hx = s.H; wa.Wx = s.W;
    wa.Cx = cin; wa.Cy = cout;
    wa.R = R; wa.S = 1; wa.pad = pad;
    wa.dw = dw;
    wa.tap_stride = (int64_t)cin * cout;
    wa.sy = cin; wa.sx = 1;
    set_wgrad(wa);
    return wa;
}

void rfi_model::conv_bn(ConvBN& c, View in, InXform xf, Shape s, const float* w, const float* w3, int R, int pad, int cin,
                        float* Y, bool train, double flops) {
    ConvArgs a = conv_same(in, xf, s, R, pad, cin, c.cout, w, w3, c.has_bias ? params + c.b_off : nullptr, Y);
    a.algo_flops = flops;
    float* ws = buf(ws_red);
    if (train) {
        a.stats = reinterpret_cast<double*>(ws);
        a.stats_max_records = (int)(bn_stats_ws_floats(c.cout) / ((size_t)c.cout * 4));
    }
    launch_conv(ctx, a);
    const int64_t M = (int64_t)s.N * s.H * s.W;
    if (train) {
        if (a.stats_records == 0) launch_bn_stats(ctx, Y, M, c.cout, ws);
        launch_bn_finalize(ctx, ws, M, c.cout, params + c.g_off, params + c.be_off, c.running_mean(), c.running_var(),
                           c.ema_repeats, c.mean(), c.invstd(), c.scale(), c.shift(), nullptr, a.stats_records);
        c.nbt += c.ema_repeats;
    } else {
        launch_bn_eval_coeffs(ctx, c.cout, params + c.g_off, params + c.be_off, c.running_mean(), c.running_var(),
                              c.scale(), c.shift());
    }
}

ConvArgs rfi_model::convt_args(const UpConv& u, View x, InXform xf, Shape s) const {
    ConvArgs a;
    a.x = x;
    a.N = s.N; a.H = s.H; a.W = s.W; a.Hin = s.H; a.Win = s.W;
    a.Cin = u.cin; a.Cout = u.cout;
    set_filters(a, params + u.w_off, u.w3);
    a.bias = params + u.b_off;
    a.Hout = 2 * s.H; a.Wout = 2 * s.W;
    a.osy = 2; a.osx = 2;
    a.R = 1; a.S = 1; a.pad = 0;
    a.zgroups = 4;
    a.xf = xf;
    return a;
}

void rfi_model::convt_backward(const UpConv& u, View dup, View x, InXform xf, Shape s, float* dx) {
    WgradArgs wa;
    wa.xop = dup;
    wa.yop = x;
    wa.xf_y = xf;
    wa.N = s.N; wa.H = s.H; wa.W = s.W; wa.Hx = 2 * s.H; wa.Wx = 2 * s.W;
    wa.Cx = u.cout; wa.Cy = u.cin;
    wa.R = 2; wa.S = 2; wa.pad = 0;
    wa.dw = grads + u.w_off;
    wa.tap_stride = (int64_t)u.cin * u.cout;
    wa.sy = 1; wa.sx = u.cin;
    set_wgrad(wa);
    wgrad_on_side(wa, nullptr);
    ConvArgs a;
    a.x = dup;
    a.N = s.N; a.H = s.H; a.W = s.W; a.Hin = 2 * s.H; a.Win = 2 * s.W;
    a.Cin = u.cout; a.Cout = u.cin;
    set_filters(a, u.wd, u.wd3);
    a.y = MutView{dx, u.cin};
    a.Hout = s.H; a.Wout = s.W;
    a.R = 2; a.S = 2; a.pad = 0;
    launch_conv(ctx, a);
}


rfi::View rfi_model::network_input(const float* x_dev, int n, int h, int w) {
    const int cp = convs[0].cin_p;
    if (cp == in_ch) return View{x_dev, in_ch};
    launch_pad_channels(ctx, x_dev, (int64_t)n * h * w, in_ch, cp, buf(x_pad));
    return View{buf(x_pad), cp};
}

void rfi_model::forward(const float* x_dev, int n, int h, int w, bool train_mode) {
    prepare(n, h, w);
    refresh_dgrad_weights();
    forward_pass(x_dev, n, h, w, train_mode);
}

void UNetModel::forward_pass(const float* x_dev, int n, int h, int w, bool train_mode) {
    if (planesP) return forward_planes(x_dev, n, h, w, train_mode);
    const int D = depth, IB = i_bott;
    auto run_conv_bn = [&](ConvBN& c, View in, InXform xf, Shape s, float* Y) {
        conv_bn(c, in, xf, s, params + c.w_off, c.w3, 3, 1, c.cin_p, Y, train_mode, 2.0 * s.N * s.H * s.W * 9.0 * c.cin * c.cout);
    };
    View cur = network_input(x_dev, n, h, w);
    if (resnet_encoder) cur = forward_resnet_encoder(cur, n, h, w, train_mode);
    else for (int l = 1; l <= D; ++l) {
        Shape s{n, h >> (l - 1), w >> (l - 1)};
        ConvBN& c1 = convs[2 * (l - 1)];
        ConvBN& c2 = convs[2 * (l - 1) + 1];
        run_conv_bn(c1, cur, InXform{}, s, buf(encY1[l]));
        if (l == 1) side_rebuild_wd();
        run_conv_bn(c2, View{buf(encY1[l]), c1.cout}, bn_xf(c1), s, buf(encY2[l]));
        launch_bn_relu_pool(ctx, buf(encY2[l]), s.N, s.H, s.W, c2.cout, c2.scale(), c2.shift(),
                            MutView{buf(concat[l]) + c2.cout, 2 * c2.cout}, buf(pool[l]), act_slope);
        cur = View{buf(pool[l]), c2.cout};
    }
    {
        Shape s{n, h >> D, w >> D};
        ConvBN& c1 = convs[IB];
        ConvBN& c2 = convs[IB + 1];
        run_conv_bn(c1, cur, InXform{}, s, buf(bottY1));
        run_conv_bn(c2, View{buf(bottY1), c1.cout}, bn_xf(c1), s, buf(bottY2));
    }
    const float* prevY = buf(bottY2);
    ConvBN* prevBN = &convs[IB + 1];
    for (int l = D; l >= 1; --l) {
        const int k = D - l;
        UpConv& u = ups[k];
        Shape sin{n, h >> l, w >> l};
        Shape s{n, h >> (l - 1), w >> (l - 1)};
        ConvArgs a = convt_args(u, View{prevY, u.cin}, bn_xf(*prevBN), sin);
        a.y = MutView{buf(concat[l]), 2 * u.cout};
        launch_conv(ctx, a);
        ConvBN& c1 = convs[IB + 2 + 2 * k];
        ConvBN& c2 = convs[IB + 2 + 2 * k + 1];
        run_conv_bn(c1, View{buf(concat[l]), 2 * u.cout}, InXform{}, s, buf(decY1[l]));
        run_conv_bn(c2, View{buf(decY1[l]), c1.cout}, bn_xf(c1), s, buf(decY2[l]));
        prevY = buf(decY2[l]);
        prevBN = &c2;
    }
    const int64_t M1 = (int64_t)n * h * w;
    launch_head_fwd(ctx, prevY, M1, feat, prevBN->scale(), prevBN->shift(), params + head_w_off,
                    params + head_b_off, out_ch, buf(logits), act_slope);
    if (head_sigmoid) launch_sigmoid_fwd(ctx, buf(logits), M1 * out_ch, buf(probs));
}

void rfi_model::loss_forward(const uint8_t* labels_dev, int n, int h, int w) {
    RFI_REQUIRE(out_ch == 1, "loss: the reference's BCE+dice step is defined for out_channels == 1");
    const int64_t cnt = (int64_t)n * h * w * out_scale * out_scale;
    if (loss_kind == 1) {
        launch_focal_reduce(ctx, buf(head_sigmoid ? probs : logits), labels_dev, cnt, focal_alpha, focal_gamma,
                            reinterpret_cast<double*>(buf(ws_red)), d_scalars);
        return;
    }
    launch_loss_reduce(ctx, buf(head_sigmoid ? probs : logits), labels_dev, cnt,
                       reinterpret_cast<double*>(buf(ws_red)), d_sums, d_scalars);
}

void rfi_model::side_begin() {
    if (!ctx->overlap) return;
    RFI_CHECK_HIP(hipEventRecord(ctx->fork_ev, ctx->main_stream));
    RFI_CHECK_HIP(hipStreamWaitEvent(ctx->side_stream, ctx->fork_ev, 0));
    ctx->stream = ctx->side_stream;
}
hipEvent_t rfi_model::next_fork_event() {
    static const bool off = getenv("RFI_NO_STOP_EVENTS") != nullptr;
    if (!ctx->overlap || off) return nullptr;
    if (ctx->fork_ring_used == ctx->fork_ring.size()) {
        hipEvent_t e;
        RFI_CHECK_HIP(hipEventCreateWithFlags(&e, hipEventDisableTiming));
        ctx->fork_ring.push_back(e);
    }
    return ctx->fork_ring[ctx->fork_ring_used++];
}
void rfi_model::side_begin_after(hipEvent_t producer_done) {
    if (!producer_done) return side_begin();
    if (!ctx->overlap) return;
    RFI_CHECK_HIP(hipStreamWaitEvent(ctx->side_stream, producer_done, 0));
    ctx->stream = ctx->side_stream;
}
void rfi_model::side_end() {
    if (!ctx->overlap) return;
    const int ring = (int)ctx->side_done.size();
    RFI_CHECK_HIP(hipEventRecord(ctx->side_done[side_seq % ring], ctx->side_stream));
    ctx->stream = ctx->main_stream;
    if (side_bound > 0 && side_seq >= side_bound)
        RFI_CHECK_HIP(hipStreamWaitEvent(ctx->main_stream, ctx->side_done[(side_seq - side_bound) % ring], 0));
    ++side_seq;
}
void rfi_model::side_join_lazy() {
    if (exchange_in_backward && ctx->exchange_active()) return side_join();
    if (!ctx->overlap || side_seq == 0) return;
    if (!lazy_ev) RFI_CHECK_HIP(hipEventCreateWithFlags(&lazy_ev, hipEventDisableTiming));
    RFI_CHECK_HIP(hipEventRecord(lazy_ev, ctx->side_stream));
    lazy_pending = true;
    side_seq = 0;
}
void rfi_model::join_pending_side() {
    if (!lazy_pending) return;
    RFI_CHECK_HIP(hipStreamWaitEvent(ctx->main_stream, lazy_ev, 0));
    lazy_pending = false;
}
void rfi_model::side_join() {
    if (!ctx->overlap || side_seq == 0) return;
    const int ring = (int)ctx->side_done.size();
    RFI_CHECK_HIP(hipStreamWaitEvent(ctx->main_stream, ctx->side_done[(side_seq - 1) % ring], 0));
    side_seq = 0;
    ctx->fork_ring_used = 0;
}

namespace rfi { void comm_bucket_allreduce(rfi_ctx* ctx, float* dptr, int64_t count); }

static hipEvent_t bucket_event(rfi_ctx* ctx) {
    if (ctx->bucket_ev_used == ctx->bucket_ev.size()) {
        hipEvent_t e;
        RFI_CHECK_HIP(hipEventCreateWithFlags(&e, hipEventDisableTiming));
        ctx->bucket_ev.push_back(e);
    }
    return ctx->bucket_ev[ctx->bucket_ev_used++];
}
void rfi_model::bucket_ready(size_t lo, size_t hi) {
    if (!exchange_in_backward || !ctx->exchange_active() || hi <= lo) return;
    static const bool no_buckets = getenv("RFI_NO_BUCKETS") != nullptr;
    const char* mf = getenv("RFI_BUCKET_MIN_FLOATS");
    const size_t min_floats = mf ? (size_t)atoll(mf) : (size_t)1 << 20;
    if (pend_hi > pend_lo) {
        RFI_REQUIRE(hi == pend_lo || lo == pend_hi, "bucket_ready: buckets must be adjacent");
        pend_lo = std::min(pend_lo, lo);
        pend_hi = std::max(pend_hi, hi);
    } else {
        pend_lo = lo;
        pend_hi = hi;
    }
    if (no_buckets) return;
    if (pend_hi - pend_lo < min_floats && pend_lo != 0) return;
    flush_bucket();
}
void rfi_model::flush_bucket() {
    if (pend_hi <= pend_lo) return;
// ... 69 lines not shown
    if (planesP) return backward_planes(x_dev, labels_dev, n, h, w);
    side_bound = resnet_encoder ? 2 : 0;
    dbias_deferred = !resnet_encoder && dbias_pool && !ctx->exchange_active();
    if (loss_kind == 1)
        launch_focal_bwd(ctx, buf(head_sigmoid ? probs : logits), labels_dev, M1, focal_alpha, focal_gamma, buf(dlogits));
    else
        launch_loss_bwd(ctx, buf(head_sigmoid ? probs : logits), labels_dev, M1, d_sums, buf(dlogits));
    if (head_sigmoid) launch_sigmoid_bwd(ctx, buf(probs), M1 * out_ch, buf(dlogits));
    int head_records = 0;
    bool head_skip = out_ch == 1;
    {
        ConvBN& last = convs[IB + 2 + 2 * (D - 1) + 1];
        const bool hdefer = dbias_deferred && head_fin_deferred;
        head_records = launch_head_bwd(ctx, buf(decY2[1]), M1, feat, last.scale(), last.shift(), params + head_w_off,
                                       out_ch, buf(dlogits), buf(gA[1]),
                                       hdefer ? dbias_pool + head_rec_off : buf(ws_red) + bn_bwd_ws_floats(M1, feat),
                                       grads + head_w_off, grads + head_b_off, act_slope, last.mean(), last.invstd(),
                                       buf(ws_red), nullptr, &head_skip, !hdefer);
    }
    for (int l = 1; l <= D; ++l) {
        const int k = D - l;
        Shape s{n, h >> (l - 1), w >> (l - 1)};
        Shape sin{n, h >> l, w >> l};
        ConvBN& c1 = convs[IB + 2 + 2 * k];
        ConvBN& c2 = convs[IB + 2 + 2 * k + 1];
        UpConv& u = ups[k];
        const bool from_head = l == 1 && head_skip;
        backward_conv_bn(this, c2, buf(gA[l]), buf(decY2[l]), View{buf(decY1[l]), c1.cout}, bn_xf(c1), s,
                         buf(gB[l]), l == 1 ? head_records : 0, from_head ? buf(dlogits) : nullptr,
                         from_head ? params + head_w_off : nullptr);
        backward_conv_bn(this, c1, buf(gB[l]), buf(decY1[l]), View{buf(concat[l]), 2 * u.cout}, InXform{}, s,
                         buf(dconcat[l]), 0);
        const float* prevY = (l == D) ? buf(bottY2) : buf(decY2[l + 1]);
        ConvBN& prevBN = (l == D) ? convs[IB + 1] : convs[IB + 2 + 2 * (k - 1) + 1];
        View dUp{buf(dconcat[l]), 2 * u.cout};
        {
            const bool defer = dbias_deferred && u.cout % 4 == 0;
            launch_channel_sum(ctx, dUp, (int64_t)s.N * s.H * s.W, u.cout, defer ? dbias_pool + u.dbias_rec_off : buf(ws_red),
                               grads + u.b_off, !defer);
        }
        convt_backward(u, dUp, View{prevY, u.cin}, bn_xf(prevBN), sin, (l == D) ? buf(gBottA) : buf(gA[l + 1]));
        bucket_ready(u.w_off, l == 1 ? n_flat : ups[k + 1].w_off);
    }
    {
        Shape s{n, h >> D, w >> D};
        ConvBN& c1 = convs[IB];
        ConvBN& c2 = convs[IB + 1];
        backward_conv_bn(this, c2, buf(gBottA), buf(bottY2), View{buf(bottY1), c1.cout}, bn_xf(c1), s, buf(gBottB), 0);
        backward_conv_bn(this, c1, buf(gBottB), buf(bottY1), View{buf(pool[D]), c1.cin}, InXform{}, s, buf(dpool[D]), 0);
        bucket_ready(c1.w_off, ups[0].w_off);
    }
    if (resnet_encoder) {
        backward_resnet_encoder(x_dev, n, h, w);
        side_join();
        return;
    }
    for (int l = D; l >= 1; --l) {
        Shape s{n, h >> (l - 1), w >> (l - 1)};
        ConvBN& c1 = convs[2 * (l - 1)];
        ConvBN& c2 = convs[2 * (l - 1) + 1];
        const std::vector<int>& gA = this->gAe;
        const std::vector<int>& gB = this->gBe;
        int have = launch_pool_bwd_merge_sums(ctx, buf(encY2[l]), s.N, s.H, s.W, c2.cout, c2.scale(), c2.shift(), c2.mean(),
                                              c2.invstd(), View{buf(dconcat[l]) + c2.cout, 2 * c2.cout}, buf(dpool[l]),
                                              buf(gA[l]), act_slope, buf(ws_red));
        if (!have)
            launch_pool_bwd_merge(ctx, buf(encY2[l]), s.N, s.H, s.W, c2.cout, c2.scale(), c2.shift(),
                                  View{buf(dconcat[l]) + c2.cout, 2 * c2.cout}, buf(dpool[l]), buf(gA[l]), act_slope);
        backward_conv_bn(this, c2, buf(gA[l]), buf(encY2[l]), View{buf(encY1[l]), c1.cout}, bn_xf(c1), s, buf(gB[l]), have);
        View in = (l == 1) ? (c1.cin_p == in_ch ? View{x_dev, in_ch} : View{buf(x_pad), c1.cin_p})
                           : View{buf(pool[l - 1]), c1.cin};
        backward_conv_bn(this, c1, buf(gB[l]), buf(encY1[l]), in, InXform{}, s,
                         (l == 1) ? nullptr : buf(dpool[l - 1]), 0);
        bucket_ready(c1.w_off, convs[l == D ? IB : 2 * l].w_off);
    }
    if (dbias_deferred) launch_finish_channel_sums_batched(ctx, static_cast<const FinishSumDesc*>(dbias_descs), dbias_n, dbias_max_c);
    side_join();
    side_bound = 2;
}

void rfi_model::apply(const rfi_hyper& hp, float grad_scale) {
    join_pending_side();
    double* ws = reinterpret_cast<double*>(buf(ws_red));
    launch_sumsq(ctx, grads, (int64_t)n_flat, ws, d_sums + 4);
    adam_step += 1;
    AdamArgs a;
    a.p = params; a.g = grads; a.m = adam_m; a.v = adam_v; a.n = (int64_t)n_flat;
    a.beta2 = (float)hp.beta2; a.eps = (float)hp.eps; a.wd = (float)hp.weight_decay;
    a.max_norm = (float)hp.max_grad_norm; a.grad_scale = grad_scale;
    a.one_minus_beta1 = (float)(1.0 - hp.beta1);
    a.one_minus_beta2 = (float)(1.0 - hp.beta2);
    a.neg_step = (float)(-(hp.lr / (1.0 - std::pow(hp.beta1, (double)adam_step))));
    a.bc2_sqrt = (float)std::sqrt(1.0 - std::pow(hp.beta2, (double)adam_step));
    a.sumsq = d_sums + 4;
    a.norm_out = d_scalars + 1;
    launch_adam(ctx, a);
    wd_dirty = true;
    x3_fresh = false;
}

void rfi_model::set_compute_dtype(int dtype) {
    arith = dtype == 1 || dtype == 4 ? Arith::BF16 : dtype == 2 || dtype == 3 ? Arith::X3 : Arith::F32;
}
void UNetModel::set_compute_dtype(int dtype) {
    rfi_model::set_compute_dtype(dtype);
    if (resnet_encoder) set_planes(dtype == 1 && feat % 16 == 0 ? 1 : 0);
    else set_planes(dtype == 1 ? 1 : (dtype == 3 ? 3 : 0));
}

void rfi_model::debug_tensor(const std::string&, const std::string&, int, bool, const float*&, size_t&) {
    throw Error("debug_tensor: this model exposes only logits / dlogits / chan (and the decoder tensors of the ResNet-encoder U-Net)");
}
void UNetModel::debug_tensor(const std::string& name, const std::string& base, int idx, bool to_host, const float*& src, size_t& n) {
    if (resnet_encoder && (base == "encY1" || base == "encY2" || base == "pool" || base == "dpool"))
        return rfi_model::debug_tensor(name, base, idx, to_host, src, n);
    RFI_REQUIRE(!(y16_flow && planesP == 1 && (base == "encY1" || base == "encY2" || base == "decY1" || base == "bottY1" ||
                                               (base == "decY2" && idx == 1))),
                "debug_tensor: this conv output is stored as bfloat16 in the bfloat16 compute mode");
    RFI_REQUIRE(!(g16_flow && planesP == 1 && (base == "gB" || base == "dpool" || base == "gBottB" || base == "gA")),
                "debug_tensor: this gradient tensor is stored as bfloat16 in the bfloat16 compute mode");
    RFI_REQUIRE(!(convt_planes && planesP == 1 && (base == "decY2" || base == "bottY2" || base == "gBottA")),
                "debug_tensor: with the transposed convs on the plane kernels this tensor is stored as bfloat16");
    const int D = depth;
    auto level = [&](const std::vector<int>& v, size_t chmul) {
        RFI_REQUIRE(idx >= 1 && idx <= D, "debug_tensor: level out of range");
        const size_t M = (size_t)pN * (pH >> (idx - 1)) * (pW >> (idx - 1));
        src = buf(v[idx]);
        n = M * ((size_t)feat << (idx - 1)) * chmul;
    };
    const size_t Mb = (size_t)pN * (pH >> D) * (pW >> D), Cb = (size_t)feat << D;
    if (base == "encY1") level(encY1, 1);
    else if (base == "encY2") level(encY2, 1);
    else if (base == "decY1") level(decY1, 1);
    else if (base == "decY2") level(decY2, 1);
    else if (base == "gA") level(!planesP && !resnet_encoder ? gAe : gA, 1);
    else if (base == "gB") level(!planesP && !resnet_encoder ? gBe : gB, 1);
    else if (base == "concat") level(concat, 2);
    else if (base == "dconcat") {
        level(dconcat, 2);
        if (convt_planes && planesP == 1 && to_host) {
            const PlaneBuf& g = pl[g16cat[idx]];
            launch_planes_to_f32(ctx, g.p, g.pstride, (int64_t)(n / ((size_t)2 * (feat << (idx - 1)))), 2 * (feat << (idx - 1)), 1,
                                 buf(dconcat[idx]), 2 * (feat << (idx - 1)));
        }
    }
    else if (base == "pool") { level(pool, 1); n /= 4; }
    else if (base == "dpool") { level(dpool, 1); n /= 4; }
    else if (base == "bottY1") { src = buf(bottY1); n = Mb * Cb; }
    else if (base == "bottY2") { src = buf(bottY2); n = Mb * Cb; }
    else if (base == "gBottA") { src = buf(gBottA); n = Mb * Cb; }
    else if (base == "gBottB") { src = buf(gBottB); n = Mb * Cb; }
    else throw Error("debug_tensor: unknown tensor " + name);
}

void UNetModel::algorithmic_flops(int n, int h, int w, double& fwd, double& step) const {
    double f = 0, stem = 0;
    for (size_t ci = 0; ci < convs.size(); ++ci) {
        const int lvl = convs[ci].level, R = convs[ci].R;
        const double M = (double)n * (h >> (lvl - 1)) * (w >> (lvl - 1));
        const double fl = 2.0 * M * R * R * convs[ci].cin * convs[ci].cout;
        f += fl;
        if (ci == 0) stem = fl;
    }
    for (int k = 0; k < depth; ++k) {
        const int l = depth - k;
        const double M = (double)n * (h >> l) * (w >> l);
        f += 2.0 * M * 4.0 * ups[k].cin * ups[k].cout;
// ... 6 lines not shown
```

rfi_toolbox_amd/csrc/model.hpp:

```cpp
#pragma once
#include "planes.hpp"

namespace rfi {

struct DevBuf {
    rfi_ctx* ctx = nullptr;
    float* p = nullptr;
    size_t n = 0;
    void ensure(rfi_ctx* c, size_t floats);
    void free();
};

struct PlaneBuf {
    rfi_ctx* ctx = nullptr;
    bf16_t* p = nullptr;
    size_t elems = 0;
    int64_t pstride = 0;
    int nchunks = 0;
    void ensure(rfi_ctx* c, int64_t pixels, int C, int P);
    void free();
};

struct ConvBN {
    std::string conv_name, bn_name;
    int cin = 0, cout = 0;
    int cin_p = 0;
    size_t w_off = 0, b_off = 0, g_off = 0, be_off = 0;
    size_t dbias_rec_off = 0;
    int ema_repeats = 1;
    int level = 1;
    int R = 3, stride = 1;
    bool has_bias = true;
    float* ws2d = nullptr;
    float* wds2d = nullptr;
    float* ws2d3 = nullptr;
    float* wds2d3 = nullptr;
    bool has_bn = true;
    bool frozen_bn = false;
    size_t chan_off = 0, wd_off = 0;
    int64_t nbt = 0;
    float* chan = nullptr;
    float* running_mean() const { return chan; }
    float* running_var() const { return chan + cout; }
    float* mean() const { return chan + 2 * cout; }
    float* invstd() const { return chan + 3 * cout; }
    float* scale() const { return chan + 4 * cout; }
    float* shift() const { return chan + 5 * cout; }
    float* c1() const { return chan + 6 * cout; }
    float* c2() const { return chan + 7 * cout; }
    float* frozen_weight() const { return mean(); }
    float* frozen_bias() const { return invstd(); }
    float* wd = nullptr;
    float* w3 = nullptr;
    float* wd3 = nullptr;
    bf16_t* wBf = nullptr;
    bf16_t* wBd = nullptr;
    bf16_t* ws3f = nullptr;
    bf16_t* ws3d = nullptr;
};

struct UpConv {
    std::string name;
    int cin = 0, cout = 0;
    size_t w_off = 0, b_off = 0;
    size_t dbias_rec_off = 0;
    size_t wd_off = 0;
    float* wd = nullptr;
    float* w3 = nullptr;
    float* wd3 = nullptr;
    bf16_t* wBf = nullptr;
    bf16_t* wBd = nullptr;
};

enum class EntryKind {
    ConvWeight,
    ConvTWeight,
    LinearWeight,
    Bias, BnWeight, BnBias,
    RunningMean, RunningVar, FrozenBnWeight, FrozenBnBias,
    NumBatchesTracked,
};
inline bool is_parameter(EntryKind k) { return k <= EntryKind::BnBias; }

struct Entry {
    std::string name;
    EntryKind kind = EntryKind::Bias;
    int ndim = 0;
    int64_t dims[4] = {0, 0, 0, 0};
    int layer = -1;
    size_t off = 0;
    int64_t numel() const {
        int64_t n = 1;
        for (int i = 0; i < ndim; ++i) n *= dims[i];
        return n;
    }
};

inline size_t align4(size_t v) { return (v + 3) & ~size_t(3); }

struct Shape { int N, H, W; };

inline InXform act_of(const ConvBN& c, float slope = 0.0f) { return act_xform(c.scale(), c.shift(), slope); }

void to_lib_conv(const float* oihw, int cout, int cin, int R, std::vector<float>& out, int cin_p = -1);
void from_lib_conv(const float* lib, int cout, int cin, int R, float* oihw, int cin_p = -1);
void to_lib_convt(const float* iohw, int cin, int cout, std::vector<float>& out);
void from_lib_convt(const float* lib, int cin, int cout, float* iohw);

}

struct rfi_model {
    rfi_ctx* ctx = nullptr;
    int in_ch = 0, out_ch = 0, feat = 0, depth = 0;
    int out_scale = 1;
    bool training = true;
    enum class Arith { F32, BF16, X3 };
    Arith arith = Arith::X3;
    bool use_w3() const { return arith == Arith::X3; }
    int planesP = 0;
    int loss_kind = 0;
    float focal_alpha = 0.25f, focal_gamma = 2.0f;
    bool head_sigmoid = false;
    int probs = -1;

    std::vector<rfi::ConvBN> convs;
    std::vector<rfi::UpConv> ups;
    size_t head_w_off = 0, head_b_off = 0;
    std::vector<rfi::Entry> entries;
    std::unordered_map<std::string, int> entry_index;

    size_t n_flat = 0;
    int64_t n_params = 0;
    float *params = nullptr, *grads = nullptr, *adam_m = nullptr, *adam_v = nullptr;
    float* grad_acc = nullptr;
    float* chan_pool = nullptr;
    float* wd_pool = nullptr;
    float* w3_pool = nullptr;
    rfi::bf16_t* ws_pool = nullptr;
    void* ws_descs = nullptr;
    int ws_n = 0;
    double ws_bytes = 0;
    std::unordered_map<const float*, const rfi::bf16_t*> ws_by_w;
    int ws_P = 0;
    int ws_need() const { return planesP ? 0 : arith == Arith::X3 ? 3 : arith == Arith::BF16 ? 1 : 0; }
    void ws_set(rfi::ConvArgs& a) const {
        auto it = ws_by_w.find(a.w);
        const rfi::bf16_t* p = it == ws_by_w.end() || ws_P != ws_need() ? nullptr : it->second;
        a.wB3 = ws_P == 3 ? p : nullptr;
        a.wB1 = ws_P == 1 ? p : nullptr;
        if (a.wB3 && x3_skipped.count(a.w)) a.w3 = nullptr;
    }
    void set_filters(rfi::ConvArgs& a, const float* w, const float* w3) const {
        a.w = w;
        a.w3 = use_w3() ? w3 : nullptr;
        ws_set(a);
        a.bf16 = arith == Arith::BF16;
        a.bf16x3 = arith == Arith::X3;
    }
    void set_wgrad(rfi::WgradArgs& wa) const {
        wa.slab = bufs[ws_slab].p;
        wa.slab_floats = bufs[ws_slab].n;
        wa.bf16 = arith == Arith::BF16;
        wa.bf16x3 = arith == Arith::X3;
    }
    bool x3_skips_ws_layers = false;
    int ws_n_fwd = 0;
    double ws_bytes_fwd = 0;
    void refresh_ws_weights(int P, int which = 0);
    hipEvent_t wd_ready = nullptr;
    bool wd_pending = false;
    bool wd_side_todo = false;
    void side_rebuild_wd();
    bool x3_reads_wd = false;
    void wait_wd();
    void* x3_descs = nullptr;
    int x3_n = 0;
    int x3_for_ws_P = -1;
    int x3_for_shape = -1;
    std::unordered_set<const float*> x3_skipped;
    double x3_bytes = 0;
    int64_t adam_step = 0;
    bool wd_dirty = true;
    bool x3_fresh = false;
    void* relayout_descs = nullptr;
    int relayout_n = 0;
    int64_t relayout_tiles = 0;
    double relayout_bytes = 0;

    int pN = 0, pH = 0, pW = 0;
    std::vector<rfi::DevBuf> bufs;
    int logits = -1, dlogits = -1;
    int x_stage = -1, x_stage2 = -1, x_pad = -1, out_stage = -1, ws_red = -1, ws_slab = -1, lab_stage = -1;
    int gx = -1;
    bool ext_dlogits = false;
    double* d_sums = nullptr;
    float* d_scalars = nullptr;
    float last_loss = 0, last_norm = 0;

    rfi_model(int in, int out, int f, int d) : in_ch(in), out_ch(out), feat(f), depth(d) {}
    virtual ~rfi_model();
    virtual void build() = 0;
    void prepare(int n, int h, int w);
    virtual void prepare_shape(int n, int h, int w) = 0;
    void forward(const float* x_dev, int n, int h, int w, bool train_mode);
    virtual void forward_pass(const float* x_dev, int n, int h, int w, bool train_mode) = 0;
    void loss_forward(const uint8_t* labels_dev, int n, int h, int w);
    void backward(const float* x_dev, const uint8_t* labels_dev, int n, int h, int w);
    virtual void backward_pass(const float* x_dev, const uint8_t* labels_dev, int n, int h, int w) = 0;
    void apply(const rfi_hyper& hp, float grad_scale);
    virtual void algorithmic_flops(int n, int h, int w, double& fwd, double& step) const = 0;
    virtual void set_compute_dtype(int dtype);
    virtual void debug_tensor(const std::string& name, const std::string& base, int idx, bool to_host, const float*& src, size_t& n);

    size_t chan_floats = 0, wd_floats = 0;
    int add_conv(rfi::ConvBN c);
    void add_up(const std::string& name, int cin, int cout);
    void add_head(const std::string& name, int cin);
    void alloc_state();
    void reset_channel_state();
    const rfi::Entry& entry(const char* name) const;
    void init_params(uint64_t seed);
    void load_entry(const rfi::Entry& e, const void* host, size_t bytes);
    void store_entry(const rfi::Entry& e, void* host, size_t bytes);
    void store_flat(const float* flat, const rfi::Entry& e, void* host, size_t bytes);
    void load_adam(const rfi::Entry& e, const void* host_m, const void* host_v, size_t bytes);
    float* buf(int i) { return bufs[i].p; }
    int new_buf() { bufs.emplace_back(); return (int)bufs.size() - 1; }
    rfi::View network_input(const float* x_dev, int n, int h, int w);
    void refresh_dgrad_weights();
    virtual bool wd_split_ok() const { return false; }
    virtual void refresh_model_weights(int which) {}

    rfi::ConvArgs conv_same(rfi::View x, rfi::InXform xf, rfi::Shape s, int R, int pad, int cin, int cout, const float* w,
                            const float* w3, const float* bias, float* y) const;
    rfi::WgradArgs wgrad_same(rfi::View x, rfi::InXform xf_x, const float* dy, rfi::Shape s, int R, int pad, int cin, int cout,
                              float* dw) const;
    void conv_bn(rfi::ConvBN& c, rfi::View in, rfi::InXform xf, rfi::Shape s, const float* w, const float* w3, int R, int pad,
                 int cin, float* Y, bool train, double flops);
    rfi::ConvArgs convt_args(const rfi::UpConv& u, rfi::View x, rfi::InXform xf, rfi::Shape s) const;
    void convt_backward(const rfi::UpConv& u, rfi::View dup, rfi::View x, rfi::InXform xf, rfi::Shape s, float* dx);

    int side_seq = 0;
    int side_bound = 2;
    void side_begin();
    hipEvent_t next_fork_event();
    void side_begin_after(hipEvent_t producer_done);
    void side_end();
    void side_join();
    hipEvent_t lazy_ev = nullptr;
    bool lazy_pending = false;
    void side_join_lazy();
    void join_pending_side();
    void wgrad_on_side(const rfi::WgradArgs& wa, hipEvent_t after, bool after_everything = false);
    bool exchange_in_backward = false;
    void bucket_ready(size_t lo, size_t hi);
    size_t pend_lo = 0, pend_hi = 0;
    void flush_bucket();
    void exchange_join();
};

namespace rfi {
struct SideScope {
    rfi_model* m;
    bool ended = false;
    explicit SideScope(rfi_model* model, hipEvent_t after = nullptr) : m(model) { m->side_begin_after(after); }
    void end() { m->side_end(); ended = true; }
    ~SideScope() { if (!ended) m->ctx->stream = m->ctx->main_stream; }
};
}

struct UNetModel : rfi_model {
    const bool resnet_encoder;
    UNetModel(int in, int out, int f, int d, bool resnet) : rfi_model(in, out, f, d), resnet_encoder(resnet) {
        x3_skips_ws_layers = !resnet;
    }
    ~UNetModel() override;
    void build() override;
    void prepare_shape(int n, int h, int w) override;
// ... 143 lines not shown
```

rfi_toolbox_amd/csrc/model_params.cpp:

```cpp
#include "model.hpp"

#include <algorithm>
#include <cmath>
#include <initializer_list>
#include <random>

using namespace rfi;

namespace rfi {

void to_lib_conv(const float* oihw, int cout, int cin, int R, std::vector<float>& out, int cin_p) {
    if (cin_p < 0) cin_p = cin;
    out.assign((size_t)R * R * cout * cin_p, 0.0f);
    for (int co = 0; co < cout; ++co)
        for (int ci = 0; ci < cin; ++ci)
            for (int t = 0; t < R * R; ++t)
                out[((size_t)t * cout + co) * cin_p + ci] = oihw[((size_t)co * cin + ci) * R * R + t];
}
void from_lib_conv(const float* lib, int cout, int cin, int R, float* oihw, int cin_p) {
    if (cin_p < 0) cin_p = cin;
    for (int co = 0; co < cout; ++co)
        for (int ci = 0; ci < cin; ++ci)
            for (int t = 0; t < R * R; ++t)
                oihw[((size_t)co * cin + ci) * R * R + t] = lib[((size_t)t * cout + co) * cin_p + ci];
// ... 8 lines not shown
void from_lib_convt(const float* lib, int cin, int cout, float* iohw) {
    for (int ci = 0; ci < cin; ++ci)
        for (int co = 0; co < cout; ++co)
            for (int t = 0; t < 4; ++t)
                iohw[((size_t)ci * cout + co) * 4 + t] = lib[((size_t)t * cout + co) * cin + ci];
}

}

namespace {

size_t flat_slot(rfi_model* m, size_t floats) {
    const size_t off = m->n_flat;
    m->n_flat = align4(m->n_flat + floats);
    return off;
}

void add_entry(rfi_model* m, const std::string& name, EntryKind kind, std::initializer_list<int64_t> dims, int layer,
               size_t off = 0) {
    Entry e;
    e.name = name;
    e.kind = kind;
    e.ndim = (int)dims.size();
    std::copy(dims.begin(), dims.end(), e.dims);
    e.layer = layer;
    e.off = off;
    if (is_parameter(kind)) m->n_params += e.numel();
    m->entry_index[name] = (int)m->entries.size();
    m->entries.push_back(e);
}

size_t lib_floats(const rfi_model* m, const Entry& e) {
    return e.kind == EntryKind::ConvWeight ? (size_t)e.dims[2] * e.dims[3] * e.dims[0] * m->convs[e.layer].cin_p : (size_t)e.numel();
}
void to_lib(const rfi_model* m, const Entry& e, const float* src, std::vector<float>& out) {
    if (e.kind == EntryKind::ConvWeight) to_lib_conv(src, (int)e.dims[0], (int)e.dims[1], (int)e.dims[2], out, m->convs[e.layer].cin_p);
    else if (e.kind == EntryKind::ConvTWeight) to_lib_convt(src, (int)e.dims[0], (int)e.dims[1], out);
    else out.assign(src, src + e.numel());
}
void from_lib(const rfi_model* m, const Entry& e, const float* lib, float* out) {
    if (e.kind == EntryKind::ConvWeight) from_lib_conv(lib, (int)e.dims[0], (int)e.dims[1], (int)e.dims[2], out, m->convs[e.layer].cin_p);
    else if (e.kind == EntryKind::ConvTWeight) from_lib_convt(lib, (int)e.dims[0], (int)e.dims[1], out);
    else std::memcpy(out, lib, (size_t)e.numel() * sizeof(float));
}

float* chan_slot(const rfi_model* m, const Entry& e) {
    switch (e.kind) {
        case EntryKind::RunningMean: return m->convs[e.layer].running_mean();
        case EntryKind::RunningVar: return m->convs[e.layer].running_var();
        case EntryKind::FrozenBnWeight: return m->convs[e.layer].frozen_weight();
        case EntryKind::FrozenBnBias: return m->convs[e.layer].frozen_bias();
        default: return nullptr;
    }
}

void check_bytes(const Entry& e, size_t bytes) {
    RFI_REQUIRE(bytes == (size_t)e.numel() * sizeof(float),
                "size mismatch for " + e.name + ": expected " + std::to_string(e.numel() * 4) + " bytes, got " +
                    std::to_string(bytes));
}

void upload(rfi_model* m, float* dst, const float* src, size_t n) {
    RFI_CHECK_HIP(hipMemcpyAsync(dst, src, n * sizeof(float), hipMemcpyHostToDevice, m->ctx->stream));
    RFI_CHECK_HIP(hipStreamSynchronize(m->ctx->stream));
}
void download(rfi_model* m, float* dst, const float* src, size_t n) {
    RFI_CHECK_HIP(hipMemcpyAsync(dst, src, n * sizeof(float), hipMemcpyDeviceToHost, m->ctx->stream));
    RFI_CHECK_HIP(hipStreamSynchronize(m->ctx->stream));
}

}

int rfi_model::add_conv(ConvBN c) {
    const int ci = (int)convs.size();
    const size_t wn = (size_t)c.R * c.R * c.cin_p * c.cout;
    const bool train_bn = c.has_bn && !c.frozen_bn;
    c.w_off = flat_slot(this, wn);
    c.b_off = flat_slot(this, c.cout);
    if (train_bn) {
        c.g_off = flat_slot(this, c.cout);
        c.be_off = flat_slot(this, c.cout);
    }
    c.chan_off = chan_floats;
    chan_floats += align4((size_t)8 * c.cout);
    c.wd_off = wd_floats;
    wd_floats += align4(wn);

    const int64_t co = c.cout;
    if (c.R == 1) {
        RFI_REQUIRE(c.cin_p == c.cin, "1x1 conv " + c.conv_name + ": padded input channels");
        add_entry(this, c.conv_name + ".weight", EntryKind::LinearWeight, {co, c.cin, 1, 1}, ci, c.w_off);
    } else {
        add_entry(this, c.conv_name + ".weight", EntryKind::ConvWeight, {co, c.cin, c.R, c.R}, ci, c.w_off);
    }
    if (c.has_bias) add_entry(this, c.conv_name + ".bias", EntryKind::Bias, {co}, ci, c.b_off);
    if (c.has_bn) {
        const std::string& bn = c.bn_name;
        if (train_bn) {
            add_entry(this, bn + ".weight", EntryKind::BnWeight, {co}, ci, c.g_off);
            add_entry(this, bn + ".bias", EntryKind::BnBias, {co}, ci, c.be_off);
        } else {
            add_entry(this, bn + ".weight", EntryKind::FrozenBnWeight, {co}, ci);
            add_entry(this, bn + ".bias", EntryKind::FrozenBnBias, {co}, ci);
        }
        add_entry(this, bn + ".running_mean", EntryKind::RunningMean, {co}, ci);
        add_entry(this, bn + ".running_var", EntryKind::RunningVar, {co}, ci);
        if (train_bn) add_entry(this, bn + ".num_batches_tracked", EntryKind::NumBatchesTracked, {}, ci);
    }
    convs.push_back(std::move(c));
    return ci;
}

void rfi_model::add_up(const std::string& name, int cin, int cout) {
    UpConv u;
    u.name = name;
    u.cin = cin;
    u.cout = cout;
    const size_t wn = (size_t)4 * cin * cout;
    u.w_off = flat_slot(this, wn);
    u.b_off = flat_slot(this, cout);
    u.wd_off = wd_floats;
    wd_floats += align4(wn);
    add_entry(this, name + ".weight", EntryKind::ConvTWeight, {cin, cout, 2, 2}, -1, u.w_off);
    add_entry(this, name + ".bias", EntryKind::Bias, {cout}, -1, u.b_off);
    ups.push_back(u);
}

void rfi_model::add_head(const std::string& name, int cin) {
    head_w_off = flat_slot(this, (size_t)out_ch * cin);
    head_b_off = flat_slot(this, out_ch);
    add_entry(this, name + ".weight", EntryKind::LinearWeight, {out_ch, cin, 1, 1}, -1, head_w_off);
    add_entry(this, name + ".bias", EntryKind::Bias, {out_ch}, -1, head_b_off);
}

void rfi_model::alloc_state() {
    ctx->activate();
    const size_t bytes = n_flat * sizeof(float);
    params = static_cast<float*>(ctx->alloc(bytes));
    grads = static_cast<float*>(ctx->alloc(bytes));
    adam_m = static_cast<float*>(ctx->alloc(bytes));
    adam_v = static_cast<float*>(ctx->alloc(bytes));
    chan_pool = static_cast<float*>(ctx->alloc(chan_floats * sizeof(float)));
    wd_pool = static_cast<float*>(ctx->alloc(wd_floats * sizeof(float)));
    d_sums = static_cast<double*>(ctx->alloc(8 * sizeof(double)));
    d_scalars = static_cast<float*>(ctx->alloc(8 * sizeof(float)));
    for (float* p : {params, grads, adam_m, adam_v}) RFI_CHECK_HIP(hipMemsetAsync(p, 0, bytes, ctx->stream));
    RFI_CHECK_HIP(hipMemsetAsync(chan_pool, 0, chan_floats * sizeof(float), ctx->stream));
    RFI_CHECK_HIP(hipMemsetAsync(d_sums, 0, 8 * sizeof(double), ctx->stream));
    RFI_CHECK_HIP(hipMemsetAsync(d_scalars, 0, 8 * sizeof(float), ctx->stream));
    for (auto& c : convs) {
        c.chan = chan_pool + c.chan_off;
        c.wd = wd_pool + c.wd_off;
    }
    for (auto& u : ups) u.wd = wd_pool + u.wd_off;
    reset_channel_state();
}

void rfi_model::reset_channel_state() {
    for (auto& c : convs) {
        std::vector<float> ch((size_t)8 * c.cout, 0.0f);
        for (int i = 0; i < c.cout; ++i) ch[c.cout + i] = 1.0f;
        if (!c.has_bn)
            for (int i = 0; i < c.cout; ++i) ch[(size_t)4 * c.cout + i] = 1.0f;
        RFI_CHECK_HIP(hipMemcpyAsync(c.chan, ch.data(), ch.size() * sizeof(float), hipMemcpyHostToDevice,
                                     ctx->stream));
        RFI_CHECK_HIP(hipStreamSynchronize(ctx->stream));
        c.nbt = 0;
    }
}

const Entry& rfi_model::entry(const char* name) const {
    RFI_REQUIRE(name, "null entry name");
    auto it = entry_index.find(name);
    RFI_REQUIRE(it != entry_index.end(), std::string("unexpected key in state_dict: ") + name);
    return entries[it->second];
}

void rfi_model::init_params(uint64_t seed) {
    std::mt19937_64 rng(seed);
    std::vector<float> flat(n_flat, 0.0f);
    auto uni = [&](float bound) {
        return (float)((std::generate_canonical<double, 53>(rng) * 2.0 - 1.0) * bound);
    };
    float last_bound = 0;
    for (const Entry& e : entries) {
        float* v = flat.data() + e.off;
        switch (e.kind) {
            case EntryKind::ConvWeight:
            case EntryKind::ConvTWeight:
            case EntryKind::LinearWeight: {
                const double fan_in = (double)e.dims[1] * e.dims[2] * e.dims[3];
                last_bound = (float)(1.0 / std::sqrt(fan_in));
                if (e.kind == EntryKind::ConvWeight) {
                    const int cin_p = convs[e.layer].cin_p, cin = (int)e.dims[1];
                    for (int64_t r = 0; r < e.dims[2] * e.dims[3] * e.dims[0]; ++r)
                        for (int ci = 0; ci < cin; ++ci) v[r * cin_p + ci] = uni(last_bound);
                } else {
                    for (int64_t i = 0; i < e.numel(); ++i) v[i] = uni(last_bound);
                }
                break;
            }
            case EntryKind::Bias:
                for (int64_t i = 0; i < e.numel(); ++i) v[i] = uni(last_bound);
                break;
            case EntryKind::BnWeight:
                std::fill(v, v + e.numel(), 1.0f);
                break;
            default:
                break;
        }
    }
    upload(this, params, flat.data(), n_flat);
    reset_channel_state();
    RFI_CHECK_HIP(hipMemsetAsync(adam_m, 0, n_flat * sizeof(float), ctx->stream));
    RFI_CHECK_HIP(hipMemsetAsync(adam_v, 0, n_flat * sizeof(float), ctx->stream));
    adam_step = 0;
    wd_dirty = true;
    x3_fresh = false;
}

void rfi_model::load_entry(const Entry& e, const void* host, size_t bytes) {
    if (e.kind == EntryKind::NumBatchesTracked) {
        RFI_REQUIRE(bytes == sizeof(int64_t), "size mismatch for " + e.name);
        convs[e.layer].nbt = *static_cast<const int64_t*>(host);
        return;
    }
    check_bytes(e, bytes);
    const float* src = static_cast<const float*>(host);
    if (float* dst = chan_slot(this, e)) {
        upload(this, dst, src, (size_t)convs[e.layer].cout);
        if (auto* b = dynamic_cast<BackboneModel*>(this)) b->frozen_dirty = true;
        return;
// ... 41 lines not shown
```

Measured before the change: 9348 patches/s.

## Fold BN, loss and grad-norm finish reductions into producer kernels via last-block tickets

Adds a last-block-done ticket scheme: each block publishes its partial reduction record with agent-scope atomic stores, bumps a per-channel-group or global ticket, and the last block to arrive performs the final reduction in the same launch. This applies to the BN statistics finalize after the workspace conv, the BCE/dice loss finish, and the gradient sum-of-squares finish, removing a separate single-block kernel launch and its dependency gap each time. The cost is extra atomics, a full vmcnt drain and barrier in every block, and a serial tail where one block finishes the reduction while the rest of the GPU idles. Tickets are stored in padded channel state and must be reset by the last block, so correctness depends on launches never being aborted midway.

```diff
diff --git a/rfi_toolbox_amd/build.py b/rfi_toolbox_amd/build.py
--- a/rfi_toolbox_amd/build.py
+++ b/rfi_toolbox_amd/build.py
@@ -15,7 +15,7 @@
 
 SOURCES = ["api.cpp", "api_ops.cpp", "model.cpp", "model_cnn.cpp", "model_planes.cpp", "model_resnet.cpp", "model_mask.cpp", "model_backbone.cpp", "model_mlp.cpp", "model_params.cpp", "elem_kernels.hip", "conv_direct.hip", "conv_mfma.hip",
            "wgrad_mfma.hip", "preprocess.hip", "synth.hip", "order_stats.hip", "planes_elem.hip", "conv_planes.hip", "conv_ws.hip", "conv_stem.hip", "gemm_ws.hip", "wgrad_ws.hip", "wgrad_stem.hip", "wgrad_planes.hip", "wgrad_split.hip", "detect_kernels.hip", "detect_sample.hip", "detect_infer.hip", "rpn_kernels.hip", "resnet_kernels.hip", "flag_stats.hip", "rfi_sim.hip", "stitch.hip", "dataset_norm.hip", "augment.hip", "sumthreshold.hip"]
-HEADERS = ["common.hpp", "kernels.hpp", "model.hpp", "planes.hpp", "ws_common.hpp", "detect_sort.hpp", "select_common.hpp", os.path.join(ROOT, "include", "rfi_hip.h")]
+HEADERS = ["common.hpp", "kernels.hpp", "model.hpp", "planes.hpp", "ws_common.hpp", "inlaunch_finish.hpp", "detect_sort.hpp", "select_common.hpp", os.path.join(ROOT, "include", "rfi_hip.h")]
 
 COMMON = ["-O3", "-std=c++17", "-fPIC", f"--offload-arch={ARCH}", "-Wall", "-Wno-unused-function",
           "-ffp-contract=off"]
diff --git a/rfi_toolbox_amd/csrc/conv_ws.hip b/rfi_toolbox_amd/csrc/conv_ws.hip
--- a/rfi_toolbox_amd/csrc/conv_ws.hip
+++ b/rfi_toolbox_amd/csrc/conv_ws.hip
@@ -4,6 +4,7 @@
 
 #include <hip/hip_ext.h>
 
+#include "inlaunch_finish.hpp"
 #include "ws_common.hpp"
 
 namespace rfi {
@@ -25,6 +26,7 @@
     float* y;
     int y_ps;
     double* stats;
+    BnFinishArgs fin;
     int wide_epi;
     unsigned long long* stamps;
 };
@@ -78,8 +80,20 @@
     const int my_tiles = (j < t_count) ? (t_count - j + gx - 1) / gx : 0;
     const int cb0 = blockIdx.y * NTL, n0 = cb0 * 32;
     double* const st_out = d.stats ? d.stats + ((size_t)blockIdx.x * d.Cout + n0) * 2 : nullptr;
+    auto finish_records = [&]() {
+        const WsDev* kd = (const WsDev*)__builtin_amdgcn_kernarg_segment_ptr();
+        asm volatile("" : "+s"(kd));
+        const BnFinishArgs f = kd->fin;
+        if (!f.tickets) return;
+        if (fin::publish_and_draw(f.tickets + blockIdx.y, (unsigned)GX, reinterpret_cast<unsigned*>(smem)))
+            fin::bn_finish_block<8>(d.stats, GX, d.Cout, n0, 32 * NTL, f, reinterpret_cast<double*>(smem + 16));
+    };
     if (my_tiles == 0) {
-        if (st_out && tid < 32 * NTL && n0 + tid < d.Cout) st_out[tid * 2] = st_out[tid * 2 + 1] = 0.0;
+        if (st_out && tid < 32 * NTL && n0 + tid < d.Cout) {
+            fin::store_record(st_out + tid * 2, 0.0);
+            fin::store_record(st_out + tid * 2 + 1, 0.0);
+        }
+        if (st_out) finish_records();
         return;
     }
     struct Tile { int n, oy0, ox0; };
@@ -499,9 +513,10 @@
                     t1 += s_stat[((w * NTL + nt) * 64 + h * 32 + cl) * 2];
                     t2 += s_stat[((w * NTL + nt) * 64 + h * 32 + cl) * 2 + 1];
                 }
-            st_out[tid * 2] = t1;
-            st_out[tid * 2 + 1] = t2;
-        }
+            fin::store_record(st_out + tid * 2, t1);
+            fin::store_record(st_out + tid * 2 + 1, t2);
+        }
+        finish_records();
     }
 }
 
@@ -519,6 +534,11 @@
     if (a.stats && GX <= a.stats_max_records) a.stats_records = GX;
     else { a.stats = nullptr; a.stats_records = 0; }
     d.stats = a.stats;
+    d.fin = BnFinishArgs{};
+    if (d.stats && a.bn_finish && a.bn_finish->tickets) {
+        d.fin = *a.bn_finish;
+        a.bn_finished = true;
+    }
     static PerDeviceOnce attr_once;
     attr_once.run(ctx->device, [&] {
         RFI_CHECK_HIP(hipFuncSetAttribute(reinterpret_cast<const void*>(&conv_ws_kernel<TB, TH, TW, NTL, XF, ADB, P>),
diff --git a/rfi_toolbox_amd/csrc/elem_kernels.hip b/rfi_toolbox_amd/csrc/elem_kernels.hip
--- a/rfi_toolbox_amd/csrc/elem_kernels.hip
+++ b/rfi_toolbox_amd/csrc/elem_kernels.hip
@@ -1,5 +1,6 @@
 #include <hip/hip_ext.h>
 
+#include "inlaunch_finish.hpp"
 #include "kernels.hpp"
 
 namespace rfi {
@@ -7,8 +8,9 @@
 namespace {
 
 constexpr int kBlock = 256;
-constexpr int kFinCh = 2;
-constexpr int kFinLanes = kBlock / kFinCh;
+using fin::kFinCh;
+using fin::kFinLanes;
+static_assert(fin::kFinBlock == kBlock, "finishing geometry");
 
 __device__ __forceinline__ double wave_sum(double v) {
 #pragma unroll
@@ -17,8 +19,7 @@
 }
 
 __device__ __forceinline__ double finish_sum(double v, double* red) {
-#pragma unroll
-    for (int o = 32; o >= kFinCh; o >>= 1) v += __shfl_xor(v, o, 64);
+    v = fin::lane_tree(v);
     const int wave = threadIdx.x >> 6, lane = threadIdx.x & 63;
     __syncthreads();
     if (lane < kFinCh) red[wave * kFinCh + lane] = v;
@@ -203,28 +204,11 @@
     s1 = finish_sum(s1, red);
     s2 = finish_sum(s2, red);
     if (rl == 0 && c < C) {
-        const double mean = s1 / count;
-        double var = s2 / count - mean * mean;
-        if (var < 0) var = 0;
-        const double invstd = 1.0 / sqrt(var + 1e-5);
-        const float meanf = (float)mean, invf = (float)invstd;
-        mean_out[c] = meanf;
-        invstd_out[c] = invf;
-        if (var_out) var_out[c] = (float)var;
-        const float sc = gamma[c] * invf;
-        scale[c] = sc;
-        shift[c] = beta[c] - meanf * sc;
-        if (running_mean) {
-            const double var_u = count > 1 ? var * (count / (count - 1.0)) : var;
-            float rm = running_mean[c], rv = running_var[c];
-            const float vuf = (float)var_u;
-            for (int k = 0; k < ema_repeats; ++k) {
-                rm = (1.0f - 0.1f) * rm + 0.1f * meanf;
-                rv = (1.0f - 0.1f) * rv + 0.1f * vuf;
-            }
-            running_mean[c] = rm;
-            running_var[c] = rv;
-        }
+        BnFinishArgs f;
+        f.running_mean = running_mean; f.running_var = running_var; f.ema_repeats = ema_repeats;
+        f.mean = mean_out; f.invstd = invstd_out; f.scale = scale; f.shift = shift; f.var_out = var_out;
+        fin::bn_finalize_channel(s1, s2, c, count, gamma[c], beta[c], running_mean ? running_mean[c] : 0.0f,
+                                 running_mean ? running_var[c] : 0.0f, f);
     }
 }
 
@@ -824,9 +808,36 @@
 
 __device__ __forceinline__ float sigmoidf_(float x) { return 1.0f / (1.0f + expf(-x)); }
 
+__device__ __forceinline__ void loss_finish_block(const double* partial, int blocks, double count, double* sums4,
+                                                  float* loss_out, double (*red)[kBlock / 64]) {
+    double s[4] = {0, 0, 0, 0};
+    for (int b = threadIdx.x; b < blocks; b += blockDim.x)
+        for (int k = 0; k < 4; ++k) s[k] += partial[(int64_t)b * 4 + k];
+    const int wave = threadIdx.x >> 6, lane = threadIdx.x & 63;
+#pragma unroll
+    for (int k = 0; k < 4; ++k) {
+        double v = wave_sum(s[k]);
+        if (lane == 0) red[k][wave] = v;
+    }
+    __syncthreads();
+    if (threadIdx.x == 0) {
+        double t[4];
+        for (int k = 0; k < 4; ++k) {
+            t[k] = 0;
+            for (int wv = 0; wv < kBlock / 64; ++wv) t[k] += red[k][wv];
+            sums4[k] = t[k];
+        }
+        const float bce = (float)(t[0] / count);
+        const float inter = (float)t[1], sp = (float)t[2], st = (float)t[3];
+        const float dice = 1.0f - (2.0f * inter + 1.0f) / (sp + st + 1.0f);
+        loss_out[0] = bce + dice;
+    }
+}
+
 __global__ void loss_reduce_kernel(const float* __restrict__ logits, const uint8_t* __restrict__ labels,
-                                   int64_t count, double* __restrict__ partial) {
+                                   int64_t count, double* partial, unsigned* ticket, double* sums4, float* loss_out) {
     __shared__ double red[4][kBlock / 64];
+    __shared__ unsigned s_last;
     double s[4] = {0, 0, 0, 0};
     for (int64_t i = (int64_t)blockIdx.x * blockDim.x + threadIdx.x; i < count;
          i += (int64_t)gridDim.x * blockDim.x) {
@@ -849,35 +860,10 @@
     if (threadIdx.x < 4) {
         double v = 0;
         for (int wv = 0; wv < kBlock / 64; ++wv) v += red[threadIdx.x][wv];
-        partial[(int64_t)blockIdx.x * 4 + threadIdx.x] = v;
-    }
-}
-
-__global__ void loss_finish_kernel(const double* __restrict__ partial, int blocks, double count,
-                                   double* __restrict__ sums4, float* __restrict__ loss_out) {
-    __shared__ double red[4][kBlock / 64];
-    double s[4] = {0, 0, 0, 0};
-    for (int b = threadIdx.x; b < blocks; b += blockDim.x)
-        for (int k = 0; k < 4; ++k) s[k] += partial[(int64_t)b * 4 + k];
-    const int wave = threadIdx.x >> 6, lane = threadIdx.x & 63;
-#pragma unroll
-    for (int k = 0; k < 4; ++k) {
-        double v = wave_sum(s[k]);
-        if (lane == 0) red[k][wave] = v;
-    }
-    __syncthreads();
-    if (threadIdx.x == 0) {
-        double t[4];
-        for (int k = 0; k < 4; ++k) {
-            t[k] = 0;
-            for (int wv = 0; wv < kBlock / 64; ++wv) t[k] += red[k][wv];
-            sums4[k] = t[k];
-        }
-        const float bce = (float)(t[0] / count);
-        const float inter = (float)t[1], sp = (float)t[2], st = (float)t[3];
-        const float dice = 1.0f - (2.0f * inter + 1.0f) / (sp + st + 1.0f);
-        loss_out[0] = bce + dice;
-    }
+        fin::store_record(partial + (int64_t)blockIdx.x * 4 + threadIdx.x, v);
+    }
+    if (fin::publish_and_draw(ticket, gridDim.x, &s_last))
+        loss_finish_block(partial, (int)gridDim.x, (double)count, sums4, loss_out, red);
 }
 
 __global__ void loss_bwd_kernel(const float* __restrict__ logits, const uint8_t* __restrict__ labels,
@@ -1213,8 +1199,9 @@
         d[i] = (float)s[i];
 }
 
-__global__ void sumsq_kernel(const float* __restrict__ g, int64_t n, double* __restrict__ partial) {
+__global__ void sumsq_kernel(const float* __restrict__ g, int64_t n, double* partial, unsigned* ticket, double* out) {
     __shared__ double red[kBlock / 64];
+    __shared__ unsigned s_last;
     double s = 0;
     const int64_t n4 = n >> 2;
     const float4* g4 = reinterpret_cast<const float4*>(g);
@@ -1233,13 +1220,11 @@
     if (threadIdx.x == 0) {
         double t = 0;
         for (int k = 0; k < kBlock / 64; ++k) t += red[k];
-        partial[blockIdx.x] = t;
-    }
-}
-__global__ void sumsq_finish_kernel(const double* __restrict__ partial, int blocks,
-                                    double* __restrict__ out) {
-    __shared__ double red[kBlock / 64];
-    double s = 0;
+        fin::store_record(partial + blockIdx.x, t);
+    }
+    if (!fin::publish_and_draw(ticket, gridDim.x, &s_last)) return;
+    const int blocks = (int)gridDim.x;
+    s = 0;
     for (int b = threadIdx.x; b < blocks; b += blockDim.x) s += partial[b];
     s = wave_sum(s);
     if ((threadIdx.x & 63) == 0) red[threadIdx.x >> 6] = s;
@@ -1629,20 +1614,12 @@
     return 4 * 1024 + 8;
 }
 void launch_loss_reduce(rfi_ctx* ctx, const float* logits, const uint8_t* labels, int64_t count,
-                        double* partial_ws, double* sums4, float* loss_out) {
+                        double* partial_ws, unsigned* ticket, double* sums4, float* loss_out) {
     int blocks = grid_for(count, 1024);
-    {
-        ProfScope ps(ctx, FAM_ELEMWISE, 0, (double)count * 5);
-        hipLaunchKernelGGL(loss_reduce_kernel, dim3(blocks), dim3(kBlock), 0, ctx->stream, logits, labels,
-                           count, partial_ws);
-        check_launch("loss_reduce");
-    }
-    {
-        ProfScope ps(ctx, FAM_ELEMWISE);
-        hipLaunchKernelGGL(loss_finish_kernel, dim3(1), dim3(kBlock), 0, ctx->stream, partial_ws, blocks,
-                           (double)count, sums4, loss_out);
-        check_launch("loss_finish");
-    }
+    ProfScope ps(ctx, FAM_ELEMWISE, 0, (double)count * 5);
+    hipLaunchKernelGGL(loss_reduce_kernel, dim3(blocks), dim3(kBlock), 0, ctx->stream, logits, labels,
+                       count, partial_ws, ticket, sums4, loss_out);
+    check_launch("loss_reduce");
 }
 void launch_focal_reduce(rfi_ctx* ctx, const float* logits, const uint8_t* labels, int64_t count, float alpha,
                          float gamma, double* partial_ws, float* loss_out) {
@@ -1802,19 +1779,11 @@
     (void)n;
     return 1024 + 8;
 }
-void launch_sumsq(rfi_ctx* ctx, const float* g, int64_t n, double* partial_ws, double* sumsq) {
+void launch_sumsq(rfi_ctx* ctx, const float* g, int64_t n, double* partial_ws, unsigned* ticket, double* sumsq) {
     int blocks = grid_for(n / 4 + 1, 1024);
-    {
-        ProfScope ps(ctx, FAM_OPTIM, 0, (double)n * 4);
-        hipLaunchKernelGGL(sumsq_kernel, dim3(blocks), dim3(kBlock), 0, ctx->stream, g, n, partial_ws);
-        check_launch("sumsq");
-    }
-    {
-        ProfScope ps(ctx, FAM_OPTIM);
-        hipLaunchKernelGGL(sumsq_finish_kernel, dim3(1), dim3(kBlock), 0, ctx->stream, partial_ws, blocks,
-                           sumsq);
-        check_launch("sumsq_finish");
-    }
+    ProfScope ps(ctx, FAM_OPTIM, 0, (double)n * 4);
+    hipLaunchKernelGGL(sumsq_kernel, dim3(blocks), dim3(kBlock), 0, ctx->stream, g, n, partial_ws, ticket, sumsq);
+    check_launch("sumsq");
 }
 void launch_adam(rfi_ctx* ctx, const AdamArgs& a) {
     ProfScope ps(ctx, FAM_OPTIM, 0, (double)a.n * 28);
diff --git a/rfi_toolbox_amd/csrc/inlaunch_finish.hpp b/rfi_toolbox_amd/csrc/inlaunch_finish.hpp
--- /dev/null
+++ b/rfi_toolbox_amd/csrc/inlaunch_finish.hpp
@@ -0,0 +1,130 @@
+#pragma once
+#include <hip/hip_runtime.h>
+
+#include "kernels.hpp"
+
+namespace rfi {
+
+namespace fin {
+
+constexpr int kFinBlock = 256;
+constexpr int kFinCh = 2;
+constexpr int kFinLanes = kFinBlock / kFinCh;
+
+__device__ __forceinline__ double lane_tree(double v) {
+#pragma unroll
+    for (int o = 32; o >= kFinCh; o >>= 1) v += __shfl_xor(v, o, 64);
+    return v;
+}
+
+__device__ __forceinline__ void store_record(double* p, double v) {
+    __hip_atomic_store(p, v, __ATOMIC_RELAXED, __HIP_MEMORY_SCOPE_AGENT);
+}
+
+__device__ __forceinline__ bool publish_and_draw(unsigned* ticket, unsigned expected, unsigned* flag) {
+    asm volatile("s_waitcnt vmcnt(0)" ::: "memory");
+    __syncthreads();
+    if (threadIdx.x == 0) {
+        const unsigned t = __hip_atomic_fetch_add(ticket, 1u, __ATOMIC_RELAXED, __HIP_MEMORY_SCOPE_AGENT);
+        const bool last = t + 1 == expected;
+        if (last) {
+            __hip_atomic_store(ticket, 0u, __ATOMIC_RELAXED, __HIP_MEMORY_SCOPE_AGENT);
+            __builtin_amdgcn_fence(__ATOMIC_ACQUIRE, "agent");
+            asm volatile("s_waitcnt vmcnt(0)" ::: "memory");
+        }
+        *flag = last ? 1u : 0u;
+    }
+    __syncthreads();
+    return *flag != 0u;
+}
+
+__device__ __forceinline__ void bn_finalize_channel(double s1, double s2, int c, double count, float gamma, float beta,
+                                                    float rm, float rv, const BnFinishArgs& f) {
+    const double mean = s1 / count;
+    double var = s2 / count - mean * mean;
+    if (var < 0) var = 0;
+    const double invstd = 1.0 / sqrt(var + 1e-5);
+    const float meanf = (float)mean, invf = (float)invstd;
+    f.mean[c] = meanf;
+    f.invstd[c] = invf;
+    if (f.var_out) f.var_out[c] = (float)var;
+    const float sc = gamma * invf;
+    f.scale[c] = sc;
+    f.shift[c] = beta - meanf * sc;
+    if (f.running_mean) {
+        const double var_u = count > 1 ? var * (count / (count - 1.0)) : var;
+        const float vuf = (float)var_u;
+        for (int k = 0; k < f.ema_repeats; ++k) {
+            rm = (1.0f - 0.1f) * rm + 0.1f * meanf;
+            rv = (1.0f - 0.1f) * rv + 0.1f * vuf;
+        }
+        f.running_mean[c] = rm;
+        f.running_var[c] = rv;
+    }
+}
+
+template <int G>
+__device__ __forceinline__ void bn_finish_block(const double* partial, int records, int C, int c0, int nch,
+                                                const BnFinishArgs& f, double* scratch) {
+    const int sub = threadIdx.x >> 8, nsub = blockDim.x >> 8, t = threadIdx.x & 255;
+    const int cl = t & (kFinCh - 1), rl = t / kFinCh, wave = t >> 6, lane = t & 63;
+    const int c_end = (c0 + nch < C) ? c0 + nch : C;
+    for (int base = c0; base < c_end; base += nsub * G * kFinCh) {
+        const int cg = base + sub * G * kFinCh;
+        const int cf = cg + t;
+        const bool fin_t = t < G * kFinCh && cf < c_end;
+        float gm = 0.0f, bt = 0.0f, rm = 0.0f, rv = 0.0f;
+        if (fin_t) {
+            gm = f.gamma[cf];
+            bt = f.beta[cf];
+            if (f.running_mean) { rm = f.running_mean[cf]; rv = f.running_var[cf]; }
+        }
+        double s1[G], s2[G];
+#pragma unroll
+        for (int g = 0; g < G; ++g) s1[g] = s2[g] = 0.0;
+        for (int r = rl; r < records; r += 2 * kFinLanes) {
+            const bool two = r + kFinLanes < records;
+            const int rb = two ? r + kFinLanes : r;
+            double2 a[G], b[G];
+#pragma unroll
+            for (int g = 0; g < G; ++g) {
+                int c = cg + g * kFinCh + cl;
+                c = c < c_end ? c : c_end - 1;
+                a[g] = *reinterpret_cast<const double2*>(partial + ((int64_t)r * C + c) * 2);
+                b[g] = *reinterpret_cast<const double2*>(partial + ((int64_t)rb * C + c) * 2);
+            }
+#pragma unroll
+            for (int g = 0; g < G; ++g) {
+                s1[g] += a[g].x;
+                s2[g] += a[g].y;
+                const double u1 = s1[g] + b[g].x, u2 = s2[g] + b[g].y;
+                s1[g] = two ? u1 : s1[g];
+                s2[g] = two ? u2 : s2[g];
+            }
+        }
+#pragma unroll
+        for (int g = 0; g < G; ++g) {
+            const double v1 = lane_tree(s1[g]), v2 = lane_tree(s2[g]);
+            if (lane < kFinCh) {
+                double* q = scratch + (((sub * G + g) * 4 + wave) * kFinCh + lane) * 2;
+                q[0] = v1;
+                q[1] = v2;
+            }
+        }
+        __syncthreads();
+        if (fin_t) {
+            const int g = t / kFinCh, l = t & (kFinCh - 1);
+            double t1 = 0, t2 = 0;
+            for (int w = 0; w < kFinBlock / 64; ++w) {
+                const double* q = scratch + (((sub * G + g) * 4 + w) * kFinCh + l) * 2;
+                t1 += q[0];
+                t2 += q[1];
+            }
+            bn_finalize_channel(t1, t2, cf, f.count, gm, bt, rm, rv, f);
+        }
+        __syncthreads();
+    }
+}
+
+}
+}
diff --git a/rfi_toolbox_amd/csrc/kernels.hpp b/rfi_toolbox_amd/csrc/kernels.hpp
--- a/rfi_toolbox_amd/csrc/kernels.hpp
+++ b/rfi_toolbox_amd/csrc/kernels.hpp
@@ -20,6 +20,21 @@
 struct MutView {
     float* p = nullptr;
     int pstride = 0;
+};
+
+struct BnFinishArgs {
+    const float* gamma = nullptr;
+    const float* beta = nullptr;
+    float* running_mean = nullptr;
+    float* running_var = nullptr;
+    int ema_repeats = 0;
+    float* mean = nullptr;
+    float* invstd = nullptr;
+    float* scale = nullptr;
+    float* shift = nullptr;
+    float* var_out = nullptr;
+    double count = 0;
+    unsigned* tickets = nullptr;
 };
 
 struct ConvArgs {
@@ -48,6 +63,8 @@
     double* stats = nullptr;
     int stats_max_records = 0;
     int stats_records = 0;
+    const BnFinishArgs* bn_finish = nullptr;
+    bool bn_finished = false;
     hipEvent_t done = nullptr;
     bool done_used = false;
 #ifdef RFI_DIAG_STAMPS
@@ -151,7 +168,7 @@
 void launch_sigmoid_fwd(rfi_ctx* ctx, const float* z, int64_t n, float* x);
 void launch_sigmoid_bwd(rfi_ctx* ctx, const float* x, int64_t n, float* d_inout);
 void launch_loss_reduce(rfi_ctx* ctx, const float* logits, const uint8_t* labels, int64_t count,
-                        double* partial_ws, double* sums4, float* loss_out);
+                        double* partial_ws, unsigned* ticket, double* sums4, float* loss_out);
 size_t loss_ws_doubles(int64_t count);
 void launch_loss_bwd(rfi_ctx* ctx, const float* logits, const uint8_t* labels, int64_t count,
                      const double* sums4, float* dlogits);
@@ -185,7 +202,7 @@
 void launch_relu_bwd(rfi_ctx* ctx, float* dA, const float* Y, int64_t n);
 void launch_pad_channels(rfi_ctx* ctx, const float* src, int64_t M, int c, int cp, float* dst);
 
-void launch_sumsq(rfi_ctx* ctx, const float* g, int64_t n, double* partial_ws, double* sumsq);
+void launch_sumsq(rfi_ctx* ctx, const float* g, int64_t n, double* partial_ws, unsigned* ticket, double* sumsq);
 size_t sumsq_ws_doubles(int64_t n);
 struct AdamArgs {
     float* p; float* g; float* m; float* v; int64_t n;
diff --git a/rfi_toolbox_amd/csrc/model.cpp b/rfi_toolbox_amd/csrc/model.cpp
--- a/rfi_toolbox_amd/csrc/model.cpp
+++ b/rfi_toolbox_amd/csrc/model.cpp
@@ -35,6 +35,7 @@
     if (x3_descs) ctx->release(x3_descs);
     if (d_sums) ctx->release(d_sums);
     if (d_scalars) ctx->release(d_scalars);
+    if (d_tickets) ctx->release(d_tickets);
     if (wd_ready) (void)hipEventDestroy(wd_ready);
     if (lazy_ev) (void)hipEventDestroy(lazy_ev);
 }
@@ -490,12 +491,20 @@
         a.stats = reinterpret_cast<double*>(ws);
         a.stats_max_records = (int)(bn_stats_ws_floats(c.cout) / ((size_t)c.cout * 4));
     }
+    const int64_t M = (int64_t)s.N * s.H * s.W;
+    BnFinishArgs fin;
+    fin.gamma = params + c.g_off; fin.beta = params + c.be_off;
+    fin.running_mean = c.running_mean(); fin.running_var = c.running_var(); fin.ema_repeats = c.ema_repeats;
+    fin.mean = c.mean(); fin.invstd = c.invstd(); fin.scale = c.scale(); fin.shift = c.shift();
+    fin.count = (double)M;
+    fin.tickets = c.tickets();
+    if (train) a.bn_finish = &fin;
     launch_conv(ctx, a);
-    const int64_t M = (int64_t)s.N * s.H * s.W;
     if (train) {
         if (a.stats_records == 0) launch_bn_stats(ctx, Y, M, c.cout, ws);
-        launch_bn_finalize(ctx, ws, M, c.cout, params + c.g_off, params + c.be_off, c.running_mean(), c.running_var(),
-                           c.ema_repeats, c.mean(), c.invstd(), c.scale(), c.shift(), nullptr, a.stats_records);
+        if (!a.bn_finished)
+            launch_bn_finalize(ctx, ws, M, c.cout, params + c.g_off, params + c.be_off, c.running_mean(), c.running_var(),
+                               c.ema_repeats, c.mean(), c.invstd(), c.scale(), c.shift(), nullptr, a.stats_records);
         c.nbt += c.ema_repeats;
     } else {
         launch_bn_eval_coeffs(ctx, c.cout, params + c.g_off, params + c.be_off, c.running_mean(), c.running_var(),
@@ -614,7 +623,7 @@
         return;
     }
     launch_loss_reduce(ctx, buf(head_sigmoid ? probs : logits), labels_dev, cnt,
-                       reinterpret_cast<double*>(buf(ws_red)), d_sums, d_scalars);
+                       reinterpret_cast<double*>(buf(ws_red)), d_tickets, d_sums, d_scalars);
 }
 
 void rfi_model::side_begin() {
@@ -850,7 +859,7 @@
 void rfi_model::apply(const rfi_hyper& hp, float grad_scale) {
     join_pending_side();
     double* ws = reinterpret_cast<double*>(buf(ws_red));
-    launch_sumsq(ctx, grads, (int64_t)n_flat, ws, d_sums + 4);
+    launch_sumsq(ctx, grads, (int64_t)n_flat, ws, d_tickets + 1, d_sums + 4);
     adam_step += 1;
     AdamArgs a;
     a.p = params; a.g = grads; a.m = adam_m; a.v = adam_v; a.n = (int64_t)n_flat;
diff --git a/rfi_toolbox_amd/csrc/model.hpp b/rfi_toolbox_amd/csrc/model.hpp
--- a/rfi_toolbox_amd/csrc/model.hpp
+++ b/rfi_toolbox_amd/csrc/model.hpp
@@ -48,6 +48,7 @@
     float* shift() const { return chan + 5 * cout; }
     float* c1() const { return chan + 6 * cout; }
     float* c2() const { return chan + 7 * cout; }
+    unsigned* tickets() const { return reinterpret_cast<unsigned*>(chan + 8 * cout); }
     float* frozen_weight() const { return mean(); }
     float* frozen_bias() const { return invstd(); }
     float* wd = nullptr;
@@ -194,6 +195,7 @@
     int gx = -1;
     bool ext_dlogits = false;
     double* d_sums = nullptr;
+    unsigned* d_tickets = nullptr;
     float* d_scalars = nullptr;
     float last_loss = 0, last_norm = 0;
 
diff --git a/rfi_toolbox_amd/csrc/model_params.cpp b/rfi_toolbox_amd/csrc/model_params.cpp
--- a/rfi_toolbox_amd/csrc/model_params.cpp
+++ b/rfi_toolbox_amd/csrc/model_params.cpp
@@ -114,7 +114,7 @@
         c.be_off = flat_slot(this, c.cout);
     }
     c.chan_off = chan_floats;
-    chan_floats += align4((size_t)8 * c.cout);
+    chan_floats += align4((size_t)8 * c.cout + (c.cout + 31) / 32);
     c.wd_off = wd_floats;
     wd_floats += align4(wn);
 
@@ -176,10 +176,12 @@
     wd_pool = static_cast<float*>(ctx->alloc(wd_floats * sizeof(float)));
     d_sums = static_cast<double*>(ctx->alloc(8 * sizeof(double)));
     d_scalars = static_cast<float*>(ctx->alloc(8 * sizeof(float)));
+    d_tickets = static_cast<unsigned*>(ctx->alloc(4 * sizeof(unsigned)));
     for (float* p : {params, grads, adam_m, adam_v}) RFI_CHECK_HIP(hipMemsetAsync(p, 0, bytes, ctx->stream));
     RFI_CHECK_HIP(hipMemsetAsync(chan_pool, 0, chan_floats * sizeof(float), ctx->stream));
     RFI_CHECK_HIP(hipMemsetAsync(d_sums, 0, 8 * sizeof(double), ctx->stream));
     RFI_CHECK_HIP(hipMemsetAsync(d_scalars, 0, 8 * sizeof(float), ctx->stream));
+    RFI_CHECK_HIP(hipMemsetAsync(d_tickets, 0, 4 * sizeof(unsigned), ctx->stream));
     for (auto& c : convs) {
         c.chan = chan_pool + c.chan_off;
         c.wd = wd_pool + c.wd_off;
```

Result: slower. 9131 patches/s (-2.3%).
